# HKUST-SING/herald

Measured on AMD Instinct MI355X. Metric: embedding rows/s (lookup+grad), higher is better.
Workload: dtype f32

## Files before the change

herald_amd/_lib.py:

```python
import ctypes
import os
import re

_PKG = os.path.dirname(os.path.abspath(__file__))
LIB_PATH = os.path.join(_PKG, "libherald_amd.so")
HEADER_PATH = os.path.join(os.path.dirname(_PKG), "include", "herald_amd.h")

_lib = None


class HeraldAmdError(RuntimeError):
    pass


class DLContext(ctypes.Structure):
    _fields_ = [("device_id", ctypes.c_int), ("device_type", ctypes.c_int)]


class DLArray(ctypes.Structure):
    _fields_ = [("data", ctypes.c_void_p), ("ctx", DLContext), ("ndim", ctypes.c_int),
                ("shape", ctypes.POINTER(ctypes.c_int64)), ("stride", ctypes.POINTER(ctypes.c_int64))]


class DLStream(ctypes.Structure):
    _fields_ = [("device_id", ctypes.c_int), ("handle", ctypes.c_void_p)]


class CacheRemote(ctypes.Structure):
    _fields_ = [("req_keys", ctypes.c_void_p), ("req_versions", ctypes.c_void_p), ("inbox_pull", ctypes.c_void_p),
                ("inbox_idx", ctypes.c_void_p), ("inbox_versions", ctypes.c_void_p), ("inbox_rows", ctypes.c_void_p),
                ("out_keys", ctypes.c_void_p), ("out_updates", ctypes.c_void_p), ("out_rows", ctypes.c_void_p),
                ("out_capacity", ctypes.c_int64), ("max_batch", ctypes.c_int64)]


class PlanView(ctypes.Structure):
    _fields_ = [("n", ctypes.c_int64), ("n_unique", ctypes.c_void_p), ("keys", ctypes.c_void_p),
                ("sorted", ctypes.c_void_p), ("perm", ctypes.c_void_p), ("inverse", ctypes.c_void_p),
                ("uniq", ctypes.c_void_p), ("counts", ctypes.c_void_p), ("seg", ctypes.c_void_p),
                ("upos", ctypes.c_void_p)]


def declared_symbols(header=None):
    text = open(header or HEADER_PATH).read()
    text = re.sub(r"/\*.*?\*/", "", text, flags=re.S)
    text = re.sub(r"\(\s*\*\s*\w+\s*\)\s*\([^;{}]*\)\s*;", ";", text)
    names = re.findall(r"\b([A-Za-z_][A-Za-z0-9_]*)\s*\([^;{}]*\)\s*;", text)
    return sorted(set(n for n in names if n not in ("defined", "int", "void", "float")))


PS_LIB_PATH = os.path.join(_PKG, "libherald_ps.so")
PS_HEADER_PATH = os.path.join(os.path.dirname(_PKG), "include", "herald_ps.h")


def load(build_if_missing=True):
    global _lib
    if _lib is not None:
        return _lib
    try:
        import torch
    except ImportError:
        pass
    if not os.path.exists(LIB_PATH):
        if not build_if_missing:
            raise HeraldAmdError("libherald_amd.so is not built (%s)" % LIB_PATH)
        from . import _build
        _build.build_lib()
    try:
        L = ctypes.CDLL(LIB_PATH, mode=ctypes.RTLD_GLOBAL)
    except OSError as e:
        raise HeraldAmdError("cannot load %s: %s" % (LIB_PATH, e))
    _declare(L)
    _lib = L
    return L


class ShardSlot(ctypes.Structure):
    _fields_ = [("world", ctypes.c_int32), ("rank", ctypes.c_int32), ("rcap", ctypes.c_int64), ("n", ctypes.c_int64),
                ("plan_ws", ctypes.c_void_p), ("keys_fixed", ctypes.c_void_p), ("meta_dev", ctypes.c_void_p),
                ("posmap", ctypes.c_void_p), ("rowmap", ctypes.c_void_p), ("counts_host", ctypes.c_void_p),
                ("owner_plan_ws", ctypes.c_void_p)]


def check(rc, what=""):
    if rc != 0:
        msg = load().ha_last_error().decode("utf-8", "replace")
        raise HeraldAmdError("%s failed: %s" % (what or "herald_amd call", msg))


def _declare(L):
    c = ctypes
    vp, i64, f32, sz = c.c_void_p, c.c_int64, c.c_float, c.c_size_t
    L.ha_version.restype = c.c_char_p
    L.ha_last_error.restype = c.c_char_p
    L.ha_device_count.restype = c.c_int
    L.ha_plan_bytes.restype = sz
    L.ha_plan_bytes.argtypes = [i64]
    L.ha_plan_view_of.argtypes = [vp, i64, c.POINTER(PlanView)]
    L.ha_plan_radix_stamps.argtypes = [vp, i64, vp, vp]
    L.ha_pend_bytes.restype = sz
    L.ha_pend_bytes.argtypes = []
    L.ha_plan_handoff_timeout.restype = vp
    L.ha_plan_handoff_timeout.argtypes = [vp]
    L.ha_step_tab_bytes.restype = sz
    L.ha_step_tab_bytes.argtypes = []
    L.ha_step_max_ids.restype = i64
    L.ha_step_max_ids.argtypes = []
    L.ha_qstep_max_ids.restype = i64
    L.ha_qstep_max_ids.argtypes = []
    L.ha_qstep_init.restype = c.c_int
    L.ha_qstep_init.argtypes = []
    L.ha_event_create.restype = vp
    L.ha_event_create.argtypes = []
    L.ha_host_unmap.restype = c.c_int
    L.ha_host_unmap.argtypes = [vp]
    L.ha_qbig_max_ids.restype = i64
    L.ha_qbig_max_ids.argtypes = []
    L.ha_xchg_create.restype = vp
    L.ha_xchg_create.argtypes = [vp, c.c_int, c.c_int]
    L.ha_qbig_plan_bytes.restype = sz
    L.ha_qbig_plan_bytes.argtypes = [i64]
    L.ha_qbig_buckets.restype = c.c_int
    L.ha_qbig_buckets.argtypes = [i64]
    L.ha_qstep_queue_bytes.restype = sz
    L.ha_qstep_queue_bytes.argtypes = [i64, i64]
    L.ha_qstep_queue_header.restype = vp
    L.ha_qstep_queue_header.argtypes = [vp]
    sigs = {
        "ha_gather_f32ids": [vp, i64, i64, vp, i64, vp, vp],
        "ha_gather_u64ids": [vp, i64, i64, vp, i64, vp, vp],
        "ha_gather_u32keys": [vp, i64, i64, vp, i64, vp, vp],
        "ha_scatter_rows_f32ids": [vp, vp, i64, i64, vp, i64, vp],
        "ha_scale_f32": [vp, i64, f32, vp],
        "ha_plan_build_f32ids": [vp, i64, vp, vp],
        "ha_plan_build_u64ids": [vp, i64, vp, vp],
        "ha_plan_build_u32keys": [vp, i64, vp, c.c_int, vp],
        "ha_plan_sort_f32ids": [vp, i64, vp, vp],
        "ha_plan_sort_u32keys": [vp, i64, vp, c.c_int, vp],
        "ha_plan_sort_u64ids": [vp, i64, vp, vp],
        "ha_plan_finish": [vp, i64, vp],
        "ha_plan_build_f32ids_lim": [vp, i64, vp, c.c_uint64, vp],
        "ha_plan_sort_f32ids_lim": [vp, i64, vp, c.c_uint64, vp],
        "ha_plan_build_u64ids_lim": [vp, i64, vp, c.c_uint64, vp],
        "ha_plan_sort_u64ids_lim": [vp, i64, vp, c.c_uint64, vp],
        "ha_plan_export_f32": [vp, i64, vp, vp, vp],
        "ha_dedup_reduce": [vp, i64, vp, i64, vp, vp],
        "ha_apply_mapped": [vp, i64, i64, vp, i64, vp, f32, vp, vp, vp, vp],
        "ha_apply_mapped2": [vp, i64, vp, i64, vp, i64, vp, f32, vp, vp, vp, vp],
        "ha_shard_bucket": [vp, i64, vp, c.c_int, vp, vp, vp],
        "ha_shard_route_f32ids": [vp, i64, vp, vp, c.c_int, vp, vp, vp],
        "ha_shard_route_u64ids": [vp, i64, vp, vp, c.c_int, vp, vp, vp],
        "ha_shard_route_pack_f32ids": [vp, i64, vp, vp, c.c_int, i64, vp, vp, vp],
        "ha_shard_route_pack_u64ids": [vp, i64, vp, vp, c.c_int, i64, vp, vp, vp],
        "ha_shard_route_unpack": [vp, c.c_int, i64, vp, vp, vp],
        "ha_shard_frames_route_f32ids": [vp, i64, vp, vp, c.c_int, i64, i64, vp, vp, vp, vp],
        "ha_shard_frames_route_u64ids": [vp, i64, vp, vp, c.c_int, i64, i64, vp, vp, vp, vp],
        "ha_shard_frames_pack": [vp, i64, vp, c.c_int, i64, i64, vp, vp, vp, vp],
        "ha_shard_frames_unpack": [vp, c.c_int, i64, i64, vp, vp, vp],
        "ha_set_tolerance_mode": [c.c_int],
        "ha_get_tolerance_mode": [],
        "ha_shard_frames_serve_push": [vp, i64, i64, vp, c.c_int, i64, vp, vp, vp],
        "ha_shard_frames_pack_batch": [vp, vp, c.c_int, vp, c.c_int, i64, i64, vp, vp, vp, vp],
        "ha_shard_frames_unpack_batch": [vp, c.c_int, c.c_int, i64, i64, vp, vp, vp],
        "ha_shard_frames_pack_batch_sized": [vp, vp, c.c_int, vp, c.c_int, c.c_int, i64, i64, vp, vp, vp, vp, vp, vp],
        "ha_shard_frames_unpack_batch_sized": [vp, c.c_int, c.c_int, i64, i64, vp, vp, vp, vp],
        "ha_shard_sized_serve_pull": [vp, i64, i64, vp, c.c_int, c.c_int, i64, vp, vp, vp],
        "ha_gather2_u32map": [vp, i64, vp, i64, i64, vp, i64, vp, vp],
        "ha_shard_sized_serve_push": [vp, i64, i64, vp, c.c_int, c.c_int, i64, vp, i64, vp, vp, vp],
        "ha_push_apply_scaled_finished": [vp, i64, i64, vp, i64, vp, f32, vp],
        "ha_qbig_plan_batch_f32ids": [vp, vp, vp, i64, i64, vp],
        "ha_qbig_plan_batch_u64ids": [vp, vp, vp, i64, i64, vp],
        "ha_qbig_queue_batch": [i64, i64, vp, vp, vp, vp, vp, i64, i64, vp, vp, vp],
        "ha_qbig_apply": [vp, i64, i64, vp, i64, vp, f32, vp, i64, vp, vp, i64, i64, c.c_uint32, vp, vp, vp],
        "ha_event_destroy": [vp],
        "ha_event_record": [vp, vp],
        "ha_stream_wait_event": [vp, vp],
        "ha_qqueue_batch_epochs": [i64, i64, vp, vp, vp, vp, vp, i64, i64, vp, vp, vp],
        "ha_shard_step_pull": [vp, i64, i64, vp, vp, vp, vp, i64, vp, vp],
        "ha_shard_step_push": [vp, i64, i64, vp, vp, vp, i64, vp, vp, f32, vp],
        "ha_shard_step": [vp, i64, i64, vp, vp, vp, vp, i64, vp, i64, vp, vp, vp, f32, vp],
        "ha_shard_steps": [vp, i64, i64, i64, vp, vp, vp, vp, i64, vp, i64, vp, vp, vp, f32, vp],
        "ha_qapply_steps_sync": [vp, i64, i64, f32, i64, i64, vp, vp, vp, vp, vp, vp, vp, vp, vp, vp, vp, vp],
        "ha_qapply_steps_counts": [vp, i64, i64, f32, i64, i64, vp, vp, vp, vp, vp, vp, vp, vp, vp, vp, vp, vp, vp],
        "ha_qapply_sync": [vp, i64, i64, vp, i64, vp, f32, vp, i64, vp, vp, i64, i64, c.c_uint32, vp, vp, vp],
        "ha_xchg_available": [],
        "ha_xchg_unique_id": [vp],
        "ha_xchg_destroy": [vp],
        "ha_xchg_bytes": [vp, vp, vp, vp, vp, vp],
        "ha_xchg_rows": [vp, vp, vp, vp, vp, i64, vp],
        "ha_qbig_plan_view": [vp, i64, vp, vp, vp, vp, vp, vp, vp],
        "ha_plan_build_batch_f32ids_lim": [vp, vp, vp, c.c_int, c.c_uint64, vp],
        "ha_plan_sort_batch_f32ids_lim": [vp, vp, vp, c.c_int, c.c_uint64, vp],
        "ha_plan_sort_batch_u64ids_lim": [vp, vp, vp, c.c_int, c.c_uint64, vp],
        "ha_plan_build_batch_u64ids_lim": [vp, vp, vp, c.c_int, c.c_uint64, vp],
        "ha_shard_frames_serve_pull": [vp, i64, i64, vp, c.c_int, i64, i64, vp, vp, vp, vp],
        "ha_shard_serve_push": [vp, i64, i64, vp, i64, vp, vp, vp],
        "ha_dedup_reduce_scaled": [vp, i64, vp, i64, f32, vp, vp],
        "ha_debug_apply_timeline": [vp, i64, i64, vp, i64, vp, f32, vp, vp],
        "ha_sgd_apply": [vp, i64, i64, vp, i64, vp, f32, vp],
        "ha_sgd_apply_finished": [vp, i64, i64, vp, i64, vp, f32, vp],
        "ha_push_apply": [vp, i64, i64, vp, i64, vp, vp],
        "ha_sgd_sparse_update_f32ids": [vp, i64, i64, vp, i64, vp, f32, vp],
        "ha_gather_sum_f32ids": [vp, i64, i64, vp, i64, i64, vp, i64, vp, vp],
        "ha_gather_sum_u64ids": [vp, i64, i64, vp, i64, i64, vp, i64, vp, vp],
        "ha_bag_of": [vp, i64, i64, vp, vp],
        "ha_sgd_apply_bags": [vp, i64, i64, vp, i64, vp, i64, vp, f32, vp],
        "ha_sgd_sparse_update_bags_f32ids": [vp, i64, i64, vp, i64, vp, i64, vp, i64, f32, vp],
        "ha_sgd_sparse_update_bags_u64ids": [vp, i64, i64, vp, i64, vp, i64, vp, i64, f32, vp],
        "ha_debug_bag_slice": [c.c_int],
        "ha_lookup_sort_f32ids": [vp, i64, i64, vp, i64, vp, vp, vp],
        "ha_lookup_sort_u64ids": [vp, i64, i64, vp, i64, vp, vp, vp],
        "ha_sgd_apply_finish": [vp, i64, i64, vp, i64, vp, f32, vp],
        "ha_push_apply_finish": [vp, i64, i64, vp, i64, vp, vp],
        "ha_sgd_apply_finish_prefetch_f32ids": [vp, i64, i64, vp, i64, vp, f32, vp, i64, vp],
        "ha_sparse_opt_fused_f32ids": [c.c_int, vp, i64, i64, vp, i64, vp, vp, vp, vp, vp, vp],
        "ha_pend_reset": [vp, vp],
        "ha_lookup_sort_pend_f32ids": [vp, i64, i64, vp, i64, vp, vp, vp, vp],
        "ha_lookup_sort_pend_u64ids": [vp, i64, i64, vp, i64, vp, vp, vp, vp],
        "ha_sgd_push_pull_f32ids": [vp, i64, i64, vp, i64, vp, f32, vp, vp, i64, vp, vp, vp, vp],
        "ha_sgd_push_pull_u64ids": [vp, i64, i64, vp, i64, vp, f32, vp, vp, i64, vp, vp, vp, vp],
        "ha_step_tab_reset": [vp, vp],
        "ha_step_f32ids": [vp, i64, i64, vp, i64, vp, f32, vp, vp, i64, vp, vp, vp, i64, vp, vp, i64, vp, vp, vp],
        "ha_step_u64ids": [vp, i64, i64, vp, i64, vp, f32, vp, vp, i64, vp, vp, vp, i64, vp, vp, i64, vp, vp, vp],
        "ha_qstep_f32ids": [vp, i64, i64, vp, i64, vp, f32, vp, i64, vp, vp, vp, i64, vp, i64, vp, i64, vp, vp],
        "ha_qstep_u64ids": [vp, i64, i64, vp, i64, vp, f32, vp, i64, vp, vp, vp, i64, vp, i64, vp, i64, vp, vp],
        "ha_qprep_f32ids": [i64, i64, vp, i64, vp, vp, i64, vp, i64, vp, i64, vp],
        "ha_qprep_u64ids": [i64, i64, vp, i64, vp, vp, i64, vp, i64, vp, i64, vp],
        "ha_qplan_batch_f32ids": [vp, vp, vp, i64, vp],
        "ha_qplan_batch_u64ids": [vp, vp, vp, i64, vp],
        "ha_qqueue_batch": [i64, i64, vp, vp, vp, vp, vp, i64, i64, vp],
        "ha_stream_gate": [vp, vp],
        "ha_debug_occupy": [i64, i64, i64, i64, vp],
        "ha_qapply": [vp, i64, i64, vp, i64, vp, f32, vp, i64, vp, vp, i64, vp],
        "ha_qapply_sized": [vp, i64, i64, vp, i64, vp, f32, vp, i64, vp, vp, i64, i64, vp],
        "ha_qapply_steps": [vp, i64, i64, f32, i64, i64, vp, vp, vp, vp, vp, vp, vp, vp, vp],
        "ha_qqueue_batch_counts": [i64, i64, vp, vp, vp, vp, vp, i64, i64, vp, vp],
        "ha_debug_qprep_f32ids": [i64, i64, vp, i64, vp, vp, i64, vp, i64, vp, i64, vp, vp],
        "ha_debug_qapply": [vp, i64, i64, vp, i64, vp, f32, vp, i64, vp, vp, i64, vp, vp],
        "ha_debug_step_fwd_timeline": [vp, i64, i64, vp, i64, vp, f32, vp, vp, i64, vp, vp, vp, i64, vp, vp, i64, vp,
                                       vp, vp, vp],
    }
    for name, args in sigs.items():
        fn = getattr(L, name)
        fn.argtypes = args
        fn.restype = c.c_int
    L.ha_cache_create.restype = vp
    L.ha_cache_create.argtypes = [c.c_int, i64, i64, i64, i64]
    L.ha_cache_destroy.restype = None
    L.ha_cache_destroy.argtypes = [vp]
    for name in ("ha_cache_data", "ha_cache_grad"):
        getattr(L, name).restype = vp
        getattr(L, name).argtypes = [vp]
    for name in ("ha_cache_limit", "ha_cache_width", "ha_cache_fused_updates"):
        getattr(L, name).restype = i64
        getattr(L, name).argtypes = [vp]
    cache_sigs = {
        "ha_cache_set_bounds": [vp, i64, i64],
        "ha_cache_set_bypass": [vp, c.c_int],
        "ha_cache_bind_store": [vp, vp, vp, i64, i64],
        "ha_cache_lookup": [vp, vp, c.c_int, i64, vp, vp],
        "ha_cache_sort_ahead": [vp, vp, c.c_int, i64, vp],
        "ha_cache_lookup_presorted": [vp, vp, c.c_int, i64, vp, vp],
        "ha_cache_sort_ahead_batch": [vp, vp, c.c_int, vp, c.c_int, vp],
        "ha_cache_plan_block": [vp, vp, c.c_int, vp, c.c_int, vp, vp],
        "ha_cache_plan_block_push_keys": [vp, vp, c.c_int, vp, vp, c.c_int, vp, c.c_int, vp, vp],
        "ha_cache_lookup_planned": [vp, i64, vp, vp],
        "ha_cache_update_planned": [vp, i64, vp, vp],
        "ha_cache_plan_pending": [vp],
        "ha_cache_run_planned_pairs": [vp, c.c_int, vp, vp, vp, vp],
        "ha_cache_plan_block_push_pull": [vp, vp, c.c_int, vp, c.c_int, vp, vp],
        "ha_cache_push_pull_planned": [vp, i64, vp, i64, vp, vp],
        "ha_cache_run_planned_push_pulls": [vp, c.c_int, vp, vp, vp, vp, vp],
        "ha_cache_update": [vp, vp, c.c_int, i64, vp, vp],
        "ha_cache_update_same_keys": [vp, i64, vp, vp],
        "ha_cache_update_with_push_keys": [vp, vp, c.c_int, i64, vp, c.c_int, i64, vp, vp],
        "ha_cache_push_pull": [vp, vp, c.c_int, i64, vp, vp, c.c_int, i64, vp, vp],
        "ha_cache_perf": [vp, vp, vp],
        "ha_cache_state": [vp, vp, vp],
        "ha_cache_phase_times": [vp, vp, vp],
        "ha_cache_set_timing": [vp, c.c_int],
        "ha_cache_stage_times": [vp, vp],
        "ha_cache_snapshot": [vp, i64, vp, vp, vp, vp, vp, vp, vp],
        "ha_cache_set_line": [vp, i64, i64, vp, vp],
        "ha_cache_set_remote": [vp],
        "ha_cache_remote_buffers": [vp, vp],
        "ha_cache_lookup_begin": [vp, vp, c.c_int, i64, vp, vp],
        "ha_cache_lookup_finish": [vp, i64, vp, vp],
        "ha_cache_outbox_count": [vp, vp, vp],
        "ha_cache_outbox_pad": [vp, i64],
        "ha_store_count_valid": [vp, i64, i64, vp, vp],
        "ha_cache_push_pull_begin": [vp, vp, c.c_int, i64, vp, c.c_int, i64, vp, vp, vp],
        "ha_cache_push_pull_finish": [vp, vp, vp],
        "ha_store_serve_sync": [vp, vp, i64, i64, vp, vp, i64, i64, vp, vp, vp, vp, vp, vp, vp],
        "ha_store_add_versions": [vp, i64, vp, vp, i64, vp],
        "ha_store_push_distinct": [vp, vp, i64, i64, vp, vp, vp, i64, vp],
    }
    for name, args in cache_sigs.items():
        fn = getattr(L, name)
        fn.argtypes = args
        fn.restype = c.c_int
    L.ha_laia_create.restype = vp
    L.ha_laia_create.argtypes = [vp, i64, i64, i64, i64, i64, i64]
    L.ha_laia_destroy.restype = None
    L.ha_laia_destroy.argtypes = [vp]
    L.ha_laia_next.restype = c.c_int
    L.ha_laia_next.argtypes = [vp, i64, i64, vp, vp, i64, vp]
    L.ha_laia_hint_next.restype = c.c_int
    L.ha_laia_hint_next.argtypes = [vp, i64]
    L.ha_laia_next_for_rank.restype = c.c_int
    L.ha_laia_next_for_rank.argtypes = [vp, i64, i64, i64, vp, vp, i64, vp]
    L.ha_laia_snapshot_keys.restype = i64
    L.ha_laia_snapshot_keys.argtypes = [vp, i64, vp, i64]
    L.ha_laia_next_topk.restype = c.c_int
    L.ha_laia_next_topk.argtypes = [vp, i64, i64, vp, i64, i64, vp, vp, i64, vp]
    L.ha_laia_counters.restype = c.c_int
    L.ha_laia_counters.argtypes = [vp, vp]
    L.ha_laia_timing.restype = c.c_int
    L.ha_laia_timing.argtypes = [vp, vp]
    L.ha_laia_timing_device.restype = c.c_int
    L.ha_laia_timing_device.argtypes = [vp, vp]
    L.ha_laia_on_device.restype = c.c_int
    L.ha_laia_on_device.argtypes = [vp]
    L.ha_shm_ring_open.restype = vp
    L.ha_shm_ring_open.argtypes = [c.c_char_p, c.c_int, i64]
    L.ha_shm_ring_close.restype = None
    L.ha_shm_ring_close.argtypes = [vp]
    L.ha_shm_ring_send.restype = c.c_int
    L.ha_shm_ring_send.argtypes = [vp, vp, i64]
    L.ha_shm_ring_recv.restype = i64
    L.ha_shm_ring_recv.argtypes = [vp, vp, i64, vp]
    L.ha_shm_ring_pending_words.restype = i64
    L.ha_shm_ring_pending_words.argtypes = [vp]
    A, S = c.POINTER(DLArray), c.POINTER(DLStream)
    dl = {
        "DLGpuEmbeddingLookUp": [A, A, A, S],
        "DLGpuEmbeddingLookUp_Gradient": [A, A, A, S],
        "IndexedSlicesOneSideAdd": [A, A, A, S],
        "DeduplicateIndexedSlices": [A, A, A, S],
        "IndexedSlices2Dense": [A, A, A, S],
        "SGDOptimizerSparseUpdate": [A, A, A, f32, S],
        "AdaGradOptimizerSparseUpdate": [A, A, A, A, f32, f32, S],
        "AdamOptimizerSparseUpdate": [A, A, A, A, A, f32, f32, f32, f32, f32, f32, S],
        "AdamWOptimizerSparseUpdate": [A, A, A, A, A, f32, f32, f32, f32, f32, f32, f32, S],
        "AddL2RegularizationSparse": [A, A, A, f32, S],
        "MomentumOptimizerSparseUpdate": [A, A, A, A, f32, f32, c.c_bool, S],
        "LambOptimizerSparseUpdate": [A, A, A, A, A, f32, f32, f32, f32, f32, f32, f32, S],
        "cpu_EmbeddingLookup": [A, A, A],
        "cpu_SGDOptimizerSparseUpdate": [A, A, A, f32],
    }
    for name, args in dl.items():
        fn = getattr(L, name)
        fn.argtypes = args
        fn.restype = c.c_int
```

herald_amd/csrc/qstep.hip:

```cpp
#include <hip/hip_ext.h>

#include "plan_dev.h"
#include "gather_dev.h"

namespace ha {

constexpr int kQMax = 7168;
#ifndef QV_GOLD
#define QV_GOLD 1
#endif
#ifndef QV_WG
#define QV_WG (QV_GOLD ? 1024 : 256)
#endif
#ifndef QV_COOPSLOTS
#define QV_COOPSLOTS (QV_GOLD ? 64 : 256)
#endif
constexpr int kQWg = QV_WG;
constexpr int kQWpw = kQWg / 64;
constexpr int kQCoopSlots = QV_COOPSLOTS;
constexpr int kQWorkerMax = 448 * 16 / kQWpw;
constexpr int kQSmallC = 3, kQSmallM = 16, kQMediumC = 15, kQLongC = 64;
enum QKind { kQS = 0, kQM = 1, kQL = 2, kQZ = 3, kQG = 4, kQNone = 15 };

struct QHeader {
// ... 1988 lines not shown
    HA_REQUIRE(rows >= 0 && rows <= 0xFFFFFFFEll && width >= 4 && width % 4 == 0 && width <= (1 << 20),
               "ha_qbig_queue_batch: rows of a multiple of 4 floats");
    HA_REQUIRE(count >= 0 && (count == 0 || (ws_a && n_a && ws_g && n_g && queues)), "ha_qbig_queue_batch: null pointer");
    HA_REQUIRE(n_cap >= 1 && n_cap <= kQBigMax, "ha_qbig_queue_batch: bad capacity");
    static DeviceOnce lds_allowed;
    if (lds_allowed.run([]() -> int {
            HA_ALLOW_LDS(qbqueue_kernel<true>, 160 * 1024);
            HA_ALLOW_LDS(qbqueue_kernel<false>, 160 * 1024);
            return 0;
        }))
        return -1;
    const int P = qbig_buckets(n_cap);
    for (int64_t k0 = 0; k0 < count; k0 += kQJoinBatch) {
        QBigJoinBatch b;
        QBigZero z;
        memset(&b, 0, sizeof(b));
        memset(&z, 0, sizeof(z));
        b.rows = static_cast<uint64_t>(rows);
        b.width = static_cast<int>(width);
        b.P = P;
        for (int64_t k = k0; k < count && b.count < kQJoinBatch; ++k) {
            HA_REQUIRE(n_a[k] >= 0 && n_g[k] >= 0 && n_a[k] <= n_cap && n_g[k] <= n_cap,
                       "ha_qbig_queue_batch: a batch is larger than the queues were sized for");
            if (n_a[k] == 0 && n_g[k] == 0)
                continue;
            HA_REQUIRE(queues[k] && (n_a[k] == 0 || ws_a[k]) && (n_g[k] == 0 || ws_g[k]),
                       "ha_qbig_queue_batch: null pointer (step %lld)", (long long)k);
            const int i = b.count++;
            if (n_a[k] > 0)
                qbig_layout(ws_a[k], n_cap, &b.a[i]);
            if (n_g[k] > 0)
                qbig_layout(ws_g[k], n_cap, &b.g[i]);
            b.a[i].n = static_cast<int>(n_a[k]);
            b.g[i].n = static_cast<int>(n_g[k]);
            const QLayout q = queue_layout(queues[k], n_cap, width);
            b.qh[i] = q.hdr;
            z.qh[z.count++] = q.hdr;
            b.mirror[i] = counts_host ? counts_host[k] : nullptr;
            b.epoch[i] = epochs ? epochs[k] : 0u;
            b.coop[i] = q.coop;
            b.wave[i] = q.wave;
            b.copy[i] = q.copy;
            b.cap_coop = q.cap_coop;
            b.cap_wave = q.cap_wave;
            b.cap_copy = q.cap_copy;
        }
        if (b.count == 0)
            continue;
        const size_t need = qjoin_lds_bytes(kQMax, kQMax), res = qjoin_lds_resident_bytes(kQMax);
        const size_t lds1 = need > res ? need : res;
        b.lds_bytes = static_cast<uint32_t>(lds1);
        hipLaunchKernelGGL(qbzero_kernel, dim3(z.count), dim3(64), 0, stream, z);
        HA_LAUNCH_CHECK();
        hipLaunchKernelGGL(qbqueue_kernel<true>, dim3(2 * (P / 4), b.count), dim3(1024), 4 * kQSubJoinLds, stream, b);
        hipLaunchKernelGGL(qbqueue_kernel<false>, dim3(2 * (P / 4), b.count), dim3(1024), lds1, stream, b);
        HA_LAUNCH_CHECK();
    }
    return 0;
}

}

using namespace ha;

extern "C" int64_t ha_qstep_max_ids(void) { return kQMax; }

extern "C" int ha_qstep_init(void) {
    const float *ids = nullptr;
    const uint64_t *ids64 = nullptr;
    if (qplan_batch<float>(&ids, nullptr, nullptr, 0, nullptr) || qplan_batch<uint64_t>(&ids64, nullptr, nullptr, 0, nullptr) ||
        qqueue_batch(0, 4, nullptr, nullptr, nullptr, nullptr, nullptr, 1, 0, nullptr))
        return -1;
    return lds_atomics_lane_ordered();
}

extern "C" size_t ha_qstep_queue_bytes(int64_t n_cap, int64_t width) {
    if (n_cap < 1 || width < 4)
        return 0;
    return queue_layout(nullptr, n_cap, width).bytes;
}

extern "C" int ha_qplan_batch_f32ids(const float *const *ids, const int64_t *n, void *const *plans, int64_t count,
                                     ha_stream_t stream) {
    return qplan_batch<float>(ids, n, plans, count, as_stream(stream));
}
extern "C" int ha_qplan_batch_u64ids(const uint64_t *const *ids, const int64_t *n, void *const *plans, int64_t count,
                                     ha_stream_t stream) {
    return qplan_batch<uint64_t>(ids, n, plans, count, as_stream(stream));
}
extern "C" int ha_qqueue_batch(int64_t rows, int64_t width, void *const *plans_a, const int64_t *n_a,
                               void *const *plans_g, const int64_t *n_g, void *const *queues, int64_t queue_n_cap,
                               int64_t count, ha_stream_t stream) {
    return qqueue_batch(rows, width, plans_a, n_a, plans_g, n_g, queues, queue_n_cap, count, as_stream(stream));
}
extern "C" int ha_qapply(float *table, int64_t rows, int64_t width, void *plan_cur, int64_t n_cur, const float *grads,
                         float lr, void *plan_next, int64_t n_next, float *next_out, const void *queue_cur,
                         int64_t queue_n_cap, ha_stream_t stream) {
    return qapply(table, rows, width, plan_cur, n_cur, grads, lr, plan_next, n_next, next_out, queue_cur, queue_n_cap,
                  as_stream(stream));
}
extern "C" int ha_qapply_sized(float *table, int64_t rows, int64_t width, void *plan_cur, int64_t n_cur, const float *grads,
                               float lr, void *plan_next, int64_t n_next, float *next_out, const void *queue_cur,
                               int64_t queue_n_cap, int64_t wave_items, ha_stream_t stream) {
    return qapply(table, rows, width, plan_cur, n_cur, grads, lr, plan_next, n_next, next_out, queue_cur, queue_n_cap,
                  as_stream(stream), nullptr, wave_items);
}
extern "C" int ha_qapply_steps(float *table, int64_t rows, int64_t width, float lr, int64_t queue_n_cap, int64_t count,
                               void *const *plan_cur, const int64_t *n_cur, const float *const *grads,
                               void *const *plan_next, const int64_t *n_next, float *const *next_out,
                               const void *const *queue_cur, const int64_t *wave_items, ha_stream_t stream) {
    HA_REQUIRE(count >= 0 && (count == 0 || (plan_cur && n_cur && grads && plan_next && n_next && next_out && queue_cur)),
               "ha_qapply_steps: null pointer");
    for (int64_t k = 0; k < count; ++k)
        if (qapply(table, rows, width, plan_cur[k], n_cur[k], grads[k], lr, plan_next[k], n_next[k], next_out[k],
                   queue_cur[k], queue_n_cap, as_stream(stream), nullptr, wave_items ? wave_items[k] : -1))
            return -1;
    return 0;
}

extern "C" void *ha_event_create(void) {
    hipEvent_t e = nullptr;
    if (hipEventCreateWithFlags(&e, hipEventDisableTiming) != hipSuccess)
        return nullptr;
    return e;
}
extern "C" int ha_event_destroy(void *event) {
    if (event)
        HA_CHECK_HIP(hipEventDestroy(static_cast<hipEvent_t>(event)));
    return 0;
}
extern "C" int ha_event_record(void *event, ha_stream_t stream) {
    HA_REQUIRE(event != nullptr, "ha_event_record: null event");
    HA_CHECK_HIP(hipEventRecord(static_cast<hipEvent_t>(event), as_stream(stream)));
    return 0;
}
extern "C" int ha_stream_wait_event(ha_stream_t stream, void *event) {
    HA_REQUIRE(event != nullptr, "ha_stream_wait_event: null event");
    HA_CHECK_HIP(hipStreamWaitEvent(as_stream(stream), static_cast<hipEvent_t>(event), 0));
    return 0;
}
extern "C" int ha_qqueue_batch_epochs(int64_t rows, int64_t width, void *const *plans_a, const int64_t *n_a,
                                      void *const *plans_g, const int64_t *n_g, void *const *queues, int64_t queue_n_cap,
                                      int64_t count, uint32_t *const *counts_host, const uint32_t *epochs,
                                      ha_stream_t stream) {
    return qqueue_batch(rows, width, plans_a, n_a, plans_g, n_g, queues, queue_n_cap, count, as_stream(stream), nullptr,
                        counts_host, epochs);
}
extern "C" int ha_qapply_steps_sync(float *table, int64_t rows, int64_t width, float lr, int64_t queue_n_cap, int64_t count,
                                    void *const *plan_cur, const int64_t *n_cur, const float *const *grads,
                                    void *const *plan_next, const int64_t *n_next, float *const *next_out,
                                    const void *const *queue_cur, const int64_t *wave_items, const uint32_t *epochs,
                                    uint32_t *err, void *done_event, ha_stream_t stream) {
    HA_REQUIRE(count >= 0 && (count == 0 || (plan_cur && n_cur && grads && plan_next && n_next && next_out && queue_cur)),
               "ha_qapply_steps_sync: null pointer");
    for (int64_t k = 0; k < count; ++k)
        if (qapply(table, rows, width, plan_cur[k], n_cur[k], grads[k], lr, plan_next[k], n_next[k], next_out[k],
                   queue_cur[k], queue_n_cap, as_stream(stream), nullptr, wave_items ? wave_items[k] : -1,
                   epochs ? epochs[k] : 0u, err, k + 1 == count ? static_cast<hipEvent_t>(done_event) : nullptr))
            return -1;
    if (count == 0 && done_event)
        HA_CHECK_HIP(hipEventRecord(static_cast<hipEvent_t>(done_event), as_stream(stream)));
    return 0;
}
extern "C" int ha_qapply_steps_counts(float *table, int64_t rows, int64_t width, float lr, int64_t queue_n_cap, int64_t count,
                                      void *const *plan_cur, const int64_t *n_cur, const float *const *grads,
                                      void *const *plan_next, const int64_t *n_next, float *const *next_out,
                                      const void *const *queue_cur, const int64_t *wave_items,
                                      const uint32_t *const *counts_host, const uint32_t *epochs, uint32_t *err,
                                      void *done_event, ha_stream_t stream) {
    (void)counts_host;
    return ha_qapply_steps_sync(table, rows, width, lr, queue_n_cap, count, plan_cur, n_cur, grads, plan_next, n_next, next_out,
                                queue_cur, wave_items, epochs, err, done_event, stream);
}
extern "C" int ha_qapply_sync(float *table, int64_t rows, int64_t width, void *plan_cur, int64_t n_cur, const float *grads,
                              float lr, void *plan_next, int64_t n_next, float *next_out, const void *queue_cur,
                              int64_t queue_n_cap, int64_t wave_items, uint32_t epoch, uint32_t *err, void *done_event,
                              ha_stream_t stream) {
    return qapply(table, rows, width, plan_cur, n_cur, grads, lr, plan_next, n_next, next_out, queue_cur, queue_n_cap,
                  as_stream(stream), nullptr, wave_items, epoch, err, static_cast<hipEvent_t>(done_event));
}

extern "C" int ha_qqueue_batch_counts(int64_t rows, int64_t width, void *const *plans_a, const int64_t *n_a,
                                      void *const *plans_g, const int64_t *n_g, void *const *queues, int64_t queue_n_cap,
                                      int64_t count, uint32_t *const *counts_host, ha_stream_t stream) {
    return qqueue_batch(rows, width, plans_a, n_a, plans_g, n_g, queues, queue_n_cap, count, as_stream(stream), nullptr,
                        counts_host);
}

template <typename IdT>
static int qprep_one(int64_t rows, int64_t width, const IdT *ahead_ids, int64_t n_ahead, void *plan_ahead, void *plan_a,
                     int64_t n_a, void *plan_g, int64_t n_g, void *queue_build, int64_t queue_n_cap, hipStream_t s) {
    if (n_ahead > 0 && qplan_batch<IdT>(&ahead_ids, &n_ahead, &plan_ahead, 1, s))
        return -1;
    if (n_a > 0 || n_g > 0)
        return qqueue_batch(rows, width, &plan_a, &n_a, &plan_g, &n_g, &queue_build, queue_n_cap, 1, s);
    return 0;
}
extern "C" int ha_qprep_f32ids(int64_t rows, int64_t width, const float *ahead_ids, int64_t n_ahead, void *plan_ahead,
                               void *plan_a, int64_t n_a, void *plan_g, int64_t n_g, void *queue_build,
                               int64_t queue_n_cap, ha_stream_t stream) {
    return qprep_one<float>(rows, width, ahead_ids, n_ahead, plan_ahead, plan_a, n_a, plan_g, n_g, queue_build,
                            queue_n_cap, as_stream(stream));
}
extern "C" int ha_qprep_u64ids(int64_t rows, int64_t width, const uint64_t *ahead_ids, int64_t n_ahead, void *plan_ahead,
                               void *plan_a, int64_t n_a, void *plan_g, int64_t n_g, void *queue_build,
                               int64_t queue_n_cap, ha_stream_t stream) {
    return qprep_one<uint64_t>(rows, width, ahead_ids, n_ahead, plan_ahead, plan_a, n_a, plan_g, n_g, queue_build,
                               queue_n_cap, as_stream(stream));
}
extern "C" int ha_qstep_f32ids(float *table, int64_t rows, int64_t width, void *plan_cur, int64_t n_cur,
                               const float *grads, float lr, void *plan_next, int64_t n_next, float *next_out,
                               const void *queue_cur, void *plan_b1, int64_t n_b1, void *queue_build,
                               int64_t queue_n_cap, const float *ahead_ids, int64_t n_ahead, void *plan_ahead,
                               ha_stream_t stream) {
    if (qprep_one<float>(rows, width, ahead_ids, n_ahead, plan_ahead, plan_next, n_next, plan_b1, n_b1, queue_build,
                         queue_n_cap, as_stream(stream)))
        return -1;
    return qapply(table, rows, width, plan_cur, n_cur, grads, lr, plan_next, n_next, next_out, queue_cur, queue_n_cap,
                  as_stream(stream));
}
extern "C" int ha_qstep_u64ids(float *table, int64_t rows, int64_t width, void *plan_cur, int64_t n_cur,
                               const float *grads, float lr, void *plan_next, int64_t n_next, float *next_out,
                               const void *queue_cur, void *plan_b1, int64_t n_b1, void *queue_build,
                               int64_t queue_n_cap, const uint64_t *ahead_ids, int64_t n_ahead, void *plan_ahead,
                               ha_stream_t stream) {
    if (qprep_one<uint64_t>(rows, width, ahead_ids, n_ahead, plan_ahead, plan_next, n_next, plan_b1, n_b1, queue_build,
                            queue_n_cap, as_stream(stream)))
        return -1;
    return qapply(table, rows, width, plan_cur, n_cur, grads, lr, plan_next, n_next, next_out, queue_cur, queue_n_cap,
                  as_stream(stream));
}

extern "C" int64_t ha_qbig_max_ids(void) { return kQBigMax; }
extern "C" size_t ha_qbig_plan_bytes(int64_t n_cap) {
    if (n_cap < 1 || n_cap > kQBigMax)
        return 0;
    return qbig_layout(nullptr, n_cap, nullptr);
}
extern "C" int ha_qbig_buckets(int64_t n_cap) { return n_cap >= 1 && n_cap <= kQBigMax ? qbig_buckets(n_cap) : 0; }
extern "C" int ha_qbig_plan_batch_f32ids(const float *const *ids, const int64_t *n, void *const *ws, int64_t n_cap,
                                         int64_t count, ha_stream_t stream) {
    return qbig_plan_batch<float>(ids, n, ws, n_cap, count, as_stream(stream));
}
extern "C" int ha_qbig_plan_batch_u64ids(const uint64_t *const *ids, const int64_t *n, void *const *ws, int64_t n_cap,
                                         int64_t count, ha_stream_t stream) {
    return qbig_plan_batch<uint64_t>(ids, n, ws, n_cap, count, as_stream(stream));
}
extern "C" int ha_qbig_queue_batch(int64_t rows, int64_t width, void *const *ws_a, const int64_t *n_a, void *const *ws_g,
                                   const int64_t *n_g, void *const *queues, int64_t n_cap, int64_t count,
                                   uint32_t *const *counts_host, const uint32_t *epochs, ha_stream_t stream) {
    return qbig_queue_batch(rows, width, ws_a, n_a, ws_g, n_g, queues, n_cap, count, counts_host, epochs, as_stream(stream));
}
extern "C" int ha_qbig_apply(float *table, int64_t rows, int64_t width, void *ws_cur, int64_t n_cur, const float *grads,
                             float lr, void *ws_next, int64_t n_next, float *next_out, const void *queue_cur, int64_t n_cap,
                             int64_t coop_items, uint32_t epoch, uint32_t *err, void *done_event, ha_stream_t stream) {
    HA_REQUIRE(n_cap >= 1 && n_cap <= kQBigMax && (n_cur == 0 || ws_cur) && (n_next == 0 || ws_next), "ha_qbig_apply: bad arguments");
    QBigRef a, g;
    memset(&a, 0, sizeof(a));
    memset(&g, 0, sizeof(g));
    if (n_cur > 0)
        qbig_layout(ws_cur, n_cap, &a);
    if (n_next > 0)
        qbig_layout(ws_next, n_cap, &g);
    return qapply_lists(table, rows, width, a.gperm, n_cur, grads, lr, g.gperm, n_next, next_out, queue_cur, n_cap, kQBigMax,
                        as_stream(stream), nullptr, -1, epoch, err, static_cast<hipEvent_t>(done_event), coop_items);
}
extern "C" int ha_qbig_plan_view(void *ws, int64_t n_cap, void **boff, void **bhdr, void **uniq, void **counts, void **seg,
                                 void **gperm, void **meta) {
    HA_REQUIRE(ws && n_cap >= 1 && n_cap <= kQBigMax, "ha_qbig_plan_view: bad arguments");
    QBigRef r;
    qbig_layout(ws, n_cap, &r);
    if (boff) *boff = r.boff;
    if (bhdr) *bhdr = r.bhdr;
    if (uniq) *uniq = r.uniq;
    if (counts) *counts = r.counts;
    if (seg) *seg = r.seg;
    if (gperm) *gperm = r.gperm;
    if (meta) *meta = r.meta;
    return 0;
}

extern "C" int ha_debug_qapply(float *table, int64_t rows, int64_t width, void *plan_cur, int64_t n_cur,
                               const float *grads, float lr, void *plan_next, int64_t n_next, float *next_out,
                               const void *queue_cur, int64_t queue_n_cap, unsigned long long *dbg, ha_stream_t stream) {
    HA_REQUIRE(dbg != nullptr, "qapply timeline: null debug buffer");
    return qapply(table, rows, width, plan_cur, n_cur, grads, lr, plan_next, n_next, next_out, queue_cur, queue_n_cap,
                  as_stream(stream), dbg);
}
extern "C" int ha_debug_qprep_f32ids(int64_t rows, int64_t width, const float *ahead_ids, int64_t n_ahead,
                                     void *plan_ahead, void *plan_a, int64_t n_a, void *plan_g, int64_t n_g,
                                     void *queue_build, int64_t queue_n_cap, unsigned long long *ph, ha_stream_t stream) {
    HA_REQUIRE(ph != nullptr, "qprep phases: null debug buffer");
    if (n_ahead > 0 && qplan_batch<float>(&ahead_ids, &n_ahead, &plan_ahead, 1, as_stream(stream), ph))
        return -1;
    if (n_a > 0 || n_g > 0)
        return qqueue_batch(rows, width, &plan_a, &n_a, &plan_g, &n_g, &queue_build, queue_n_cap, 1, as_stream(stream),
                            ph + 16);
    return 0;
}

extern "C" const uint32_t *ha_qstep_queue_header(const void *queue) {
    return reinterpret_cast<const uint32_t *>(queue);
}
```

herald_amd/ops.py:

```python
import ctypes
import os

import numpy as np

import torch

from . import _lib
from ._lib import DLArray, DLContext, DLStream, PlanView, check


def _stream_ptr(stream=None):
    if stream is None:
        return ctypes.c_void_p(torch._C._cuda_getCurrentRawStream(torch.cuda.current_device()))
    if isinstance(stream, int):
        return ctypes.c_void_p(stream)
    return ctypes.c_void_p(stream.cuda_stream)


def _ptr(t):
    return ctypes.c_void_p(t.data_ptr())


def _raw_stream(stream=None):
    p = _stream_ptr(stream).value
# ... 404 lines not shown
    L = _lib.load()
    _require(table, torch.float32, "table")
    n = ids.numel()
    width = table.shape[1]
    if n > plan.capacity:
        raise ValueError("plan capacity %d < %d ids" % (plan.capacity, n))
    if out is None:
        out = torch.empty(tuple(ids.shape) + (width,), dtype=torch.float32, device=table.device)
    fn = getattr(L, "ha_lookup_sort_pend_" + _ids_kind(ids))
    check(fn(_ptr(table), table.shape[0], width, _ptr(ids), n, _ptr(out), _ptr(plan.ws), _ptr(pend.buf),
             _stream_ptr(stream)), "ha_lookup_sort_pend")
    plan.n = n
    plan._view = None
    plan.produced_on(stream)
    return out


def sgd_push_pull(table, plan_cur, grads, lr, pend_cur, next_ids=None, plan_next=None, pend_next=None,
                  next_out=None, stream=None):
    L = _lib.load()
    _require(table, torch.float32, "table")
    _require(grads, torch.float32, "grads")
    width = table.shape[1]
    if next_ids is None:
        check(L.ha_sgd_push_pull_f32ids(_ptr(table), table.shape[0], width, _ptr(plan_cur.ws), plan_cur.n,
                                        _ptr(grads), ctypes.c_float(lr), _ptr(pend_cur.buf), None, 0, None,
                                        None, None, _stream_ptr(stream)), "ha_sgd_push_pull")
        plan_cur.produced_on(stream)
        return None
    n = next_ids.numel()
    if n > plan_next.capacity:
        raise ValueError("plan capacity %d < %d ids" % (plan_next.capacity, n))
    if next_out is None:
        next_out = torch.empty(tuple(next_ids.shape) + (width,), dtype=torch.float32, device=table.device)
    fn = getattr(L, "ha_sgd_push_pull_" + _ids_kind(next_ids))
    check(fn(_ptr(table), table.shape[0], width, _ptr(plan_cur.ws), plan_cur.n, _ptr(grads),
             ctypes.c_float(lr), _ptr(pend_cur.buf), _ptr(next_ids), n, _ptr(next_out), _ptr(plan_next.ws),
             _ptr(pend_next.buf), _stream_ptr(stream)), "ha_sgd_push_pull")
    plan_next.n = n
    plan_next._view = None
    plan_cur.produced_on(stream)
    plan_next.produced_on(stream)
    return next_out


def check_handoff(plans):
    for p in plans:
        p._sync_producer()
        p._raise_if_handoff_timed_out()


class SortAhead:

    def __init__(self, table, capacity, lr, device=None):
        _require(table, torch.float32, "table")
        self.table, self.lr = table, float(lr)
        self.device = table.device if device is None else torch.device(device)
        self.plans = [IndexPlan(capacity, self.device), IndexPlan(capacity, self.device)]
        self.side = torch.cuda.Stream(device=self.device)
        self.k = 0
        self.plan = None

    def _sort(self, plan, ids):
        cur = torch.cuda.current_stream(self.device)
        self.side.wait_stream(cur)
        plan.sort(ids.reshape(-1), stream=self.side, key_limit=self.table.shape[0])

    def begin(self, ids0):
        self.k = 0
        self._sort(self.plans[0], ids0)
        torch.cuda.current_stream(self.device).wait_stream(self.side)

    def lookup(self, ids, next_ids=None, out=None):
        if next_ids is not None:
            self._sort(self.plans[(self.k + 1) % 2], next_ids)
        return embedding_lookup(self.table, ids, out=out)

    def apply(self, grads):
        cur = torch.cuda.current_stream(self.device)
        plan = self.plans[self.k % 2]
        sgd_apply_finish(self.table, plan, grads, self.lr)
        cur.wait_stream(self.side)
        self.plan = plan
        self.k += 1
        return plan


def step_max_ids():
    return int(_lib.load().ha_step_max_ids())


class StepPipeline:

    NPLAN, NTAB = 4, 4

    def __init__(self, table, capacity, lr, device=None):
        L = _lib.load()
        _require(table, torch.float32, "table")
        self.table, self.lr = table, float(lr)
        self.device = table.device if device is None else torch.device(device)
        if capacity > step_max_ids():
            raise ValueError("ha_step_* takes at most %d ids per batch (got capacity %d): use sgd_push_pull / "
                             "lookup_sort + sgd_apply_finish" % (step_max_ids(), capacity))
        self.capacity = capacity
        self.plans = [IndexPlan(capacity, self.device) for _ in range(self.NPLAN)]
        self.tab_bytes = int(L.ha_step_tab_bytes())
        self.tabs = torch.empty(self.NTAB * self.tab_bytes, dtype=torch.uint8, device=self.device)
        self.c = None
        self.n = {}
        self.shape = {}
        self.reset()

    def _tab(self, c):
        return self.tabs.data_ptr() + (c % self.NTAB) * self.tab_bytes

    def plan_of(self, c):
        return self.plans[c % self.NPLAN]

    def reset(self, stream=None):
        L = _lib.load()
        for t in range(self.NTAB):
            check(L.ha_step_tab_reset(self._tab(t), _stream_ptr(stream)), "ha_step_tab_reset")
        if stream is None:
            torch.cuda.current_stream(self.device).synchronize()
        self.c, self.n, self.shape = None, {}, {}
        return self

    def launch(self, c, n_cur, grads, n_next, out, n_fin, ahead_ids, stream=None):
        L = _lib.load()
        t = self.table
        width = t.shape[1]
        n_ahead = 0 if ahead_ids is None else ahead_ids.numel()
        if max(n_cur, n_next, n_fin, n_ahead) > self.capacity:
            raise ValueError("plan capacity %d < %d ids" % (self.capacity, max(n_cur, n_next, n_fin, n_ahead)))
        if n_cur:
            _require(grads, torch.float32, "grads")
            if grads.numel() != n_cur * width:
                raise ValueError("grads must hold %d x %d values" % (n_cur, width))
        if n_next:
            _require(out, torch.float32, "out")
            if out.numel() != n_next * width:
                raise ValueError("out must hold %d x %d values" % (n_next, width))
        kind = _ids_kind(ahead_ids) if n_ahead else "f32ids"
        fn = getattr(L, "ha_step_" + kind)
        check(fn(_ptr(t), t.shape[0], width,
                 _ptr(self.plan_of(c).ws) if n_cur else None, n_cur, _ptr(grads) if n_cur else None,
                 ctypes.c_float(self.lr), self._tab(c) if n_cur else None,
                 _ptr(self.plan_of(c + 1).ws) if n_next else None, n_next, _ptr(out) if n_next else None,
                 self._tab(c + 1) if n_next else None,
                 _ptr(self.plan_of(c + 2).ws) if n_fin else None, n_fin, self._tab(c + 2) if n_fin else None,
                 _ptr(ahead_ids) if n_ahead else None, n_ahead,
                 _ptr(self.plan_of(c + 3).ws) if n_ahead else None,
                 self._tab(c + 3), _stream_ptr(stream)), "ha_step")
        if n_fin:
            self.plan_of(c + 2).produced_on(stream)
        if n_ahead:
            pl = self.plan_of(c + 3)
            pl.n = n_ahead
            pl._view = None
            pl.produced_on(stream)

    def _call(self, c, grads, ahead_ids, out, stream):
        n_cur, n_next, n_fin = self.n.get(c, 0), self.n.get(c + 1, 0), self.n.get(c + 2, 0)
        n_ahead = 0 if ahead_ids is None else ahead_ids.numel()
        if n_next and out is None:
            out = torch.empty(tuple(self.shape[c + 1]) + (self.table.shape[1],), dtype=torch.float32,
                              device=self.table.device)
        self.launch(c, n_cur, grads, n_next, out, n_fin, ahead_ids, stream)
        if n_cur:
            del self.n[c]
        if n_ahead:
            self.n[c + 3] = n_ahead
            self.shape[c + 3] = tuple(ahead_ids.shape)
        self.c = c + 1
        return out if n_next else None

    def start(self, ids0, ids1=None, ids2=None, out=None, stream=None):
        self._call(-3, None, ids0, None, stream)
        self._call(-2, None, ids1, None, stream)
        return self._call(-1, None, ids2, out, stream)

    def step(self, grads, ahead_ids=None, out=None, stream=None):
        if self.c is None or self.c not in self.n:
            raise RuntimeError("StepPipeline.step without a batch in flight (call start first)")
        return self._call(self.c, grads, ahead_ids, out, stream)


def qbig_max_ids():
    return int(_lib.load().ha_qbig_max_ids())


class WidePlan:

    def __init__(self, capacity, device):
        L = _lib.load()
        self.capacity, self.device = int(capacity), device
        self.ws = torch.zeros(int(L.ha_qbig_plan_bytes(self.capacity)), dtype=torch.uint8, device=device)
        torch.cuda.current_stream(device).synchronize()
        self.buckets = int(L.ha_qbig_buckets(self.capacity))
        self.n = 0
        self._produced_on, self._view = 0, None

    def groups(self):
        L = _lib.load()
        ptr = [ctypes.c_void_p() for _ in range(7)]
        check(L.ha_qbig_plan_view(_ptr(self.ws), self.capacity, *[ctypes.byref(p) for p in ptr]), "ha_qbig_plan_view")
        torch.cuda.synchronize(self.device)
        base = self.ws.data_ptr()

        def arr(p, count, dtype):
            off = p.value - base
            return self.ws[off:off + count * dtype.itemsize].view(dtype).cpu().numpy()
        P, n = self.buckets, self.n
        boff = arr(ptr[0], P + 1, torch.int32).astype(np.int64)
        hdr = arr(ptr[1], P * 32, torch.int64).reshape(P, 32)
        uniq = arr(ptr[2], max(n, 1), torch.int32).astype(np.int64) & 0xFFFFFFFF
        counts = arr(ptr[3], max(n, 1), torch.int32).astype(np.int64)
        gperm = arr(ptr[5], max(n, 1), torch.int32).astype(np.int64)
        meta = arr(ptr[6], 1, torch.int32)
        keys, cnts, lists = [], [], []
        for p in range(P):
            U = int(hdr[p, 0])
            o = int(boff[p])
            keys.append(uniq[o:o + U])
            cnts.append(counts[o:o + U])
            lists.append(gperm[o:int(boff[p + 1])])
        return {"overflow": int(meta[0]), "bucket_sizes": np.diff(boff), "uniq": np.concatenate(keys) if keys else uniq[:0],
                "counts": np.concatenate(cnts) if cnts else counts[:0], "perm": np.concatenate(lists) if lists else gperm[:0]}


def qstep_max_ids():
    return int(_lib.load().ha_qstep_max_ids())


class SortAheadPipeline:

    NBLOCKS = 3

    def __init__(self, table, max_ids, lr, block=8, key_limit=None, device=None, finish_ahead=None):
        _require(table, torch.float32, "table")
        self.table, self.lr, self.block = table, float(lr), int(block)
        self.device = table.device if device is None else torch.device(device)
        self.key_limit = int(table.shape[0]) if key_limit is None else int(key_limit)
        self.finish_ahead = bool(finish_ahead)
        self.plans = [[IndexPlan(max_ids, self.device) for _ in range(self.block)] for _ in range(self.NBLOCKS)]
        self.side = torch.cuda.Stream(device=self.device)
        self._sorted = [torch.cuda.Event() for _ in range(self.NBLOCKS)]
        self._freed = [None] * self.NBLOCKS
        self._first = [0] * self.NBLOCKS
        self._count = [0] * self.NBLOCKS
        self._next_block = 0
        self._waited = -1

    def prepare_block(self, ids_list):
        if not 0 < len(ids_list) <= self.block:
            raise ValueError("a block holds 1..%d batches" % self.block)
        b = self._next_block
        slot = b % self.NBLOCKS
        self.side.wait_stream(torch.cuda.current_stream(self.device))
        with torch.cuda.stream(self.side):
            if self._freed[slot] is not None:
                self.side.wait_event(self._freed[slot])
            for i, ids in enumerate(ids_list):
                if self.finish_ahead:
                    self.plans[slot][i].build(ids, stream=self.side, key_limit=self.key_limit)
                else:
                    self.plans[slot][i].sort(ids, stream=self.side, key_limit=self.key_limit)
            self._sorted[slot].record(self.side)
        self._first[slot] = (self._first[(b - 1) % self.NBLOCKS] + self._count[(b - 1) % self.NBLOCKS]) if b else 0
        self._count[slot] = len(ids_list)
        self._next_block = b + 1
        return b

    def _plan(self, k, stream):
        for b in range(max(self._next_block - self.NBLOCKS, 0), self._next_block):
            slot = b % self.NBLOCKS
            if self._first[slot] <= k < self._first[slot] + self._count[slot]:
                if b > self._waited:
                    (stream or torch.cuda.current_stream(self.device)).wait_event(self._sorted[slot])
                    self._waited = b
                return slot, k - self._first[slot]
        raise ValueError("step %d is not in a prepared block" % k)

    def lookup(self, k, ids, out=None, stream=None):
        self._plan(k, stream)
        return embedding_lookup(self.table, ids, out=out, stream=stream)

    def apply(self, k, grads, stream=None):
        slot, i = self._plan(k, stream)
        if self.finish_ahead:
            sgd_apply(self.table, self.plans[slot][i], grads, self.lr, stream=stream, finished=True)
            self.plans[slot][i].produced_on(self.side)
        else:
            sgd_apply_finish(self.table, self.plans[slot][i], grads, self.lr, stream=stream)
        if i == self._count[slot] - 1:
            ev = torch.cuda.Event()
            ev.record(stream or torch.cuda.current_stream(self.device))
            self._freed[slot] = ev
        return self.plans[slot][i]


class QueueStepPipeline:

    def __init__(self, table, capacity, lr, device=None, block=8, overlap=True, sync="events", min_flags_block=8):
        L = _lib.load()
        _require(table, torch.float32, "table")
        self.table, self.lr = table, float(lr)
        self.device = table.device if device is None else torch.device(device)
        self.wide = capacity > qstep_max_ids()
        if capacity > qbig_max_ids():
            raise ValueError("ha_qstep_* takes at most %d ids per batch (got capacity %d): use SortAheadPipeline / "
                             "lookup_sort + sgd_apply_finish" % (qbig_max_ids(), capacity))
        if table.shape[1] % 4 != 0:
            raise ValueError("ha_qstep_* needs rows of a multiple of 4 floats")
        with torch.cuda.device(self.device):
            if L.ha_qstep_init() < 0:
                check(-1, "ha_qstep_init")
        self.capacity = max(int(capacity), 1)
        self.overlap = bool(overlap)
        if sync not in ("events", "flags"):
            raise ValueError("sync must be 'events' or 'flags'")
        self.sync = sync if self.overlap else "events"
        if self.sync == "flags" and int(block) < int(min_flags_block):
            self.sync = "events"
        self._done_ev, self._cev_pool = {}, []
        self._cev_busy = []
        self.block = int(block) if self.overlap else 1
        if not 1 <= self.block <= 64:
            raise ValueError("block must be 1..64")
        self.LOOKAHEAD = 3 * self.block
        self.NPLAN, self.NQUEUE = 4 * self.block, 2 * self.block
        self.ROTATION = 4 * self.block
        self.plans = [(WidePlan if self.wide else IndexPlan)(self.capacity, self.device) for _ in range(self.NPLAN)]
        self.queue_bytes = int(L.ha_qstep_queue_bytes(self.capacity, table.shape[1]))
        self.queues = torch.zeros(self.NQUEUE * self.queue_bytes, dtype=torch.uint8, device=self.device)
        torch.cuda.current_stream(self.device).synchronize()
        side_prio = 0
        if os.environ.get("HA_QSIDE_PRIO") in ("low", "high"):
            try:
                lo_hi = torch.cuda.Stream.priority_range()
                side_prio = max(lo_hi) if os.environ["HA_QSIDE_PRIO"] == "low" else min(lo_hi)
            except Exception:
                side_prio = 0
        self.side = torch.cuda.Stream(device=self.device, priority=side_prio) if self.overlap else None
        self.COUNTS = 8192
        self.counts = torch.zeros((self.COUNTS, 4), dtype=torch.int32).pin_memory()
        self._counts_np = self.counts.numpy()
        self._counts_c = (ctypes.c_int32 * (self.COUNTS * 4)).from_address(self.counts.data_ptr())
        self._counts_base = self.counts.data_ptr()
        self._L = L
        self._plan_ptr = [p.ws.data_ptr() for p in self.plans]
        self._queue_ptr = [self.queues.data_ptr() + q * self.queue_bytes for q in range(self.NQUEUE)]
        self._ev_pool = []
        self._last_items = 0
        self.fallbacks, self._fb_plan, self._wide_ids = 0, None, {}
        self._enq_last = None
        self.reset()

    def close(self):
        for ev in list(self._done_ev.values()) + self._cev_pool + [e for e, _ in self._cev_busy]:
            self._L.ha_event_destroy(ev)
        self._done_ev, self._cev_pool, self._cev_busy = {}, [], []

    def __del__(self):
        try:
            self.close()
        except Exception:
            pass

    def reset(self, stream=None):
        if self._done_ev:
            if self.side is not None:
                marker = self._event() if hasattr(self, "_ev_pool") else torch.cuda.Event()
                marker.record(self.side)
                self._cev_busy.extend((e, marker) for e in self._done_ev.values())
            else:
                self._cev_pool.extend(self._done_ev.values())
        self._done_ev = {}
        self.c, self.n, self.shape, self.ids = None, {}, {}, {}
        self._enq_last, self._covered = None, -(1 << 60)
        self._ev_side = {}
        self._held = {}
        return self

    def plan_of(self, b):
        return self.plans[b % self.NPLAN]

    def _queue(self, c):
        return self.queues.data_ptr() + (c % self.NQUEUE) * self.queue_bytes

    def queue_header(self, c):
        off = (c % self.NQUEUE) * self.queue_bytes
        torch.cuda.synchronize(self.device)
        h = self.queues[off:off + 40].view(torch.int32).cpu().tolist()
        d = dict(zip(("wave_items", "workgroup_items", "long", "medium", "small", "copy_items"), h))
        d["overflow"] = int(h[8] != 0 or h[9] != 0)
        return d

    def overflowed(self):
        return bool((self._counts_np[:, 3] & ~4).any())

    def _raise_if_failed(self, steps):
        cc, ring = self._counts_c, self.COUNTS
        for j in steps:
            f = cc[4 * (j % ring) + 3]
            if f & ~4:
                raise RuntimeError("QueueStepPipeline: step %d failed on the device (flags %d: 1 = queue overflow, 2 = an "
                                   "occurrence list out of position order, 8 = an apply launch gave up waiting -- its queue was "
                                   "never completed, or an item it depends on never finished; the table is partly updated)"
                                   % (j, f))

    def prepare_block(self, b, ids_of, stream=None, ph=None):
        L = self._L
        rows, width = self.table.shape
        main = stream if stream is not None else torch.cuda.current_stream(self.device)
        B = self.block
        s = self.side if self.overlap else main
        sp = _stream_ptr(s)
        vp, i64 = ctypes.c_void_p, ctypes.c_int64
        flags = self.sync == "flags"
        self._raise_if_failed(range(max((b - 2) * B, 0), max((b - 1) * B, 0)))
        if self.overlap and flags:
            cev = self._done_ev.pop(b - 1, None)
            if cev is not None:
                check(L.ha_stream_wait_event(sp, cev), "ha_stream_wait_event")
                marker = self._event()
                marker.record(s)
                self._cev_busy.append((cev, marker))
                self._covered = b * B - 1
            elif self._enq_last is not None and self._enq_last > self._covered:
                ev = self._event()
                ev.record(main)
                s.wait_event(ev)
                self._ev_pool.append(ev)
                self._covered = self._enq_last
        elif self.overlap:
            ev = self._event()
            ev.record(main)
            s.wait_event(ev)
        sel = {"f32ids": [], "u64ids": []}
        held = []
        for j in range((b + 2) * B, (b + 3) * B):
            t = ids_of(j)
            if t is None:
                continue
            m = t.numel()
            if m == 0:
                continue
            if m > self.capacity:
                raise ValueError("plan capacity %d < %d ids" % (self.capacity, m))
            if not t.is_cuda or not t.is_contiguous():
                raise ValueError("ids must be contiguous device tensors")
            sel[_ids_kind(t)].append((j, t, m))
            held.append(t)
            self.n[j] = m
            if self.wide:
                self._wide_ids[j] = t
                self._wide_ids.pop(j - 5 * B, None)
        for kind, lst in sel.items():
            if not lst:
                continue
            cnt = len(lst)
            ids_arr = (vp * cnt)(*[t.data_ptr() for _, t, _ in lst])
            n_arr = (i64 * cnt)(*[m for _, _, m in lst])
            pl_arr = (vp * cnt)(*[self._plan_ptr[j % self.NPLAN] for j, _, _ in lst])
            if ph is not None and kind == "f32ids":
                j0, t0, m0 = lst[0]
                check(L.ha_debug_qprep_f32ids(rows, width, _ptr(t0), m0, _ptr(self.plan_of(j0).ws), None, 0,
                                              None, 0, None, self.capacity, _ptr(ph), sp), "ha_debug_qprep")
            if self.wide:
                check(getattr(L, "ha_qbig_plan_batch_" + kind)(ids_arr, n_arr, pl_arr, self.capacity, cnt, sp),
                      "ha_qbig_plan_batch")
            else:
                check(getattr(L, "ha_qplan_batch_" + kind)(ids_arr, n_arr, pl_arr, cnt, sp), "ha_qplan_batch")
            for j, _, m in lst:
                pl = self.plans[j % self.NPLAN]
                pl.n = m
                pl._view = None
                pl._produced_on = sp.value if sp.value is not None else 0
        self._held[b] = held
        self._held.pop(b - 2, None)
        nget = self.n.get
        steps = [j for j in range((b + 1) * B, (b + 2) * B) if nget(j, 0) or nget(j + 1, 0)]
        if steps:
            cnt = len(steps)
            pp, NP, NQ = self._plan_ptr, self.NPLAN, self.NQUEUE
            pa = (vp * cnt)(*[pp[j % NP] if nget(j, 0) else None for j in steps])
            na = (i64 * cnt)(*[nget(j, 0) for j in steps])
            pg = (vp * cnt)(*[pp[(j + 1) % NP] if nget(j + 1, 0) else None for j in steps])
            ng = (i64 * cnt)(*[nget(j + 1, 0) for j in steps])
            qs = (vp * cnt)(*[self._queue_ptr[j % NQ] for j in steps])
            if ph is not None:
                check(L.ha_debug_qprep_f32ids(rows, width, None, 0, None, pa[0], na[0], pg[0], ng[0], qs[0], self.capacity,
                                              _ptr(ph), sp), "ha_debug_qprep")
            base, ring, cc = self._counts_base, self.COUNTS, self._counts_c
            for j in steps:
                at = 4 * (j % ring)
                cc[at] = 0
                cc[at + 2] = 0
                cc[at + 3] &= ~4
            cs = (vp * cnt)(*[base + 16 * (j % ring) for j in steps])
            eps = (ctypes.c_uint32 * cnt)(*[self._epoch(j) for j in steps])
            if self.wide:
                check(L.ha_qbig_queue_batch(rows, width, pa, na, pg, ng, qs, self.capacity, cnt, cs, eps, sp),
                      "ha_qbig_queue_batch")
            else:
                check(L.ha_qqueue_batch_epochs(rows, width, pa, na, pg, ng, qs, self.capacity, cnt, cs, eps, sp),
                      "ha_qqueue_batch")
        if self.overlap and not flags:
            ev = self._event()
            ev.record(s)
            self._ev_side[b] = ev
            ready = self._ev_side.pop(b - 1, None)
            if ready is not None:
                main.wait_event(ready)
                self._ev_pool.append(ready)

    def _event(self):
        return self._ev_pool.pop() if self._ev_pool else torch.cuda.Event()

    @staticmethod
    def _epoch(j):
        return (j + (1 << 24)) & 0xFFFFFFFF

    def _block_done_event(self, c):
        if self.sync != "flags" or (c + 1) % self.block != 0:
            return None
        if not self._cev_pool and self._cev_busy and self._cev_busy[0][1].query():
            old_ev, marker = self._cev_busy.pop(0)
            self._ev_pool.append(marker)
            self._cev_pool.append(old_ev)
        ev = self._cev_pool.pop() if self._cev_pool else ctypes.c_void_p(self._L.ha_event_create())
        if not ev:
            raise RuntimeError("ha_event_create failed")
        old = self._done_ev.pop(c // self.block, None)
        if old is not None:
            self._cev_pool.append(old)
        self._done_ev[c // self.block] = ev
        return ev

    def _err_ptr(self, c):
        return ctypes.c_void_p(self._counts_base + 16 * (c % self.COUNTS) + 12)

    def wave_items(self, c):
        at = 4 * (c % self.COUNTS)
        if self._counts_c[at + 3]:
            raise RuntimeError("ha_qqueue_batch: the work queue of step %d is unusable (flags %d: 1 = overflow, 2 = an "
                               "occurrence list out of position order, 4 = a hash bucket of a wide batch holds more than "
                               "%d ids)" % (c, self._counts_c[at + 3], qstep_max_ids()))
        if os.environ.get("HA_QHINT") == "0":
            return -1
        w, cp = self._counts_c[at], self._counts_c[at + 2]
        return w + cp - 2 if w > 0 and cp > 0 else -1

    def apply(self, c, grads, out, stream=None, dbg=None, n_cur=None, n_next=None):
        L = self._L
        t = self.table
        rows, width = t.shape
        n_cur = self.n.get(c, 0) if n_cur is None else int(n_cur)
        n_next = self.n.get(c + 1, 0) if n_next is None else int(n_next)
        if n_cur:
            _require(grads, torch.float32, "grads")
            if grads.numel() != n_cur * width:
                raise ValueError("grads must hold %d x %d values" % (n_cur, width))
        if n_next:
            _require(out, torch.float32, "out")
            if out.numel() != n_next * width:
                raise ValueError("out must hold %d x %d values" % (n_next, width))
        flags = self.sync == "flags" and dbg is None
        capturing = flags and torch.cuda.is_current_stream_capturing()
        if capturing:
            raise RuntimeError("QueueStepPipeline(sync='flags'): steps cannot be captured into a hipGraph (use sync='events')")
        done = self._block_done_event(c) if flags else None
        self._enq_last = c if self._enq_last is None else max(self._enq_last, c)
        if not (n_cur or n_next):
            if done is not None:
                check(L.ha_event_record(done, _stream_ptr(stream)), "ha_event_record")
            return
        args = [_ptr(t), rows, width, _ptr(self.plan_of(c).ws) if n_cur else None, n_cur,
                _ptr(grads) if n_cur else None, ctypes.c_float(self.lr),
                _ptr(self.plan_of(c + 1).ws) if n_next else None, n_next, _ptr(out) if n_next else None,
                self._queue(c), self.capacity]
        if self.wide:
            flag, coop = self._wide_built(c)
            if flag & 4:
                self._wide_fallback(c, grads, out, stream, n_cur, n_next, done)
                return
            if flag:
                self.wave_items(c)
            check(L.ha_qbig_apply(*args, coop, self._epoch(c) if flags else 0, self._err_ptr(c) if flags else None, done,
                                  _stream_ptr(stream)), "ha_qbig_apply")
        elif flags:
            check(L.ha_qapply_sync(*args, self.wave_items(c), self._epoch(c), self._err_ptr(c), done, _stream_ptr(stream)),
                  "ha_qapply_sync")
        elif dbg is None:
            check(L.ha_qapply_sized(*args, self.wave_items(c), _stream_ptr(stream)), "ha_qapply")
        else:
            check(L.ha_debug_qapply(*args, _ptr(dbg), _stream_ptr(stream)), "ha_debug_qapply")

    def _wide_built(self, c, timeout=20.0):
        import time
        at = 4 * (c % self.COUNTS)
        cc = self._counts_c
        if cc[at] == 0:
            t0 = time.perf_counter()
            while cc[at] == 0:
                if time.perf_counter() - t0 > timeout:
                    raise RuntimeError("QueueStepPipeline: the queue of step %d was not built within %.0f s (was its block "
                                       "prepared?)" % (c, timeout))
        return cc[at + 3], max(cc[at + 1] - 1, 0)

    def _wide_fallback(self, c, grads, out, stream, n_cur, n_next, done):
        self.fallbacks += 1
        if n_cur:
            if self._fb_plan is None:
                self._fb_plan = IndexPlan(self.capacity, self.device)
            self._fb_plan.build(self._wide_ids[c], stream=stream)
            sgd_apply(self.table, self._fb_plan, grads.reshape(n_cur, -1), self.lr, stream=stream, finished=True)
        if n_next:
            embedding_lookup(self.table, self._wide_ids[c + 1].reshape(-1), out=out.reshape(n_next, -1), stream=stream)
        if done is not None:
            check(self._L.ha_event_record(done, _stream_ptr(stream)), "ha_event_record")

    def apply_call(self, c, grads, out, stream, n_cur, n_next, sized=True):
        if self.sync == "flags":
            raise RuntimeError("apply_call: use apply / apply_steps_call with sync='flags'")
        L = self._L
        t = self.table
        rows, width = t.shape
        hint = ctypes.c_int64(-1)
        args = (ctypes.c_void_p(t.data_ptr()), ctypes.c_int64(rows), ctypes.c_int64(width),
                ctypes.c_void_p(self.plan_of(c).ws.data_ptr() if n_cur else None), ctypes.c_int64(n_cur),
                ctypes.c_void_p(grads.data_ptr() if n_cur else None), ctypes.c_float(self.lr),
                ctypes.c_void_p(self.plan_of(c + 1).ws.data_ptr() if n_next else None), ctypes.c_int64(n_next),
                ctypes.c_void_p(out.data_ptr() if n_next else None), ctypes.c_void_p(self._queue(c)),
                ctypes.c_int64(self.capacity), hint, _stream_ptr(stream))
        fn = L.ha_qapply_sized

        def call(k):
            self._enq_last = k if self._enq_last is None else max(self._enq_last, k)
            if sized:
                hint.value = self.wave_items(k)
            if fn(*args) != 0:
                check(-1, "ha_qapply")
        return call

    def apply_steps_call(self, c0, grads_list, out_list, stream, n, sized=True):
        L = self._L
        t = self.table
        rows, width = t.shape
        cnt = len(grads_list)
        vp, i64 = ctypes.c_void_p, ctypes.c_int64
        pc = (vp * cnt)(*[self.plan_of(c0 + i).ws.data_ptr() for i in range(cnt)])
        pn = (vp * cnt)(*[self.plan_of(c0 + i + 1).ws.data_ptr() for i in range(cnt)])
        ns = (i64 * cnt)(*[n] * cnt)
        gs = (vp * cnt)(*[g.data_ptr() for g in grads_list])
        os_ = (vp * cnt)(*[o.data_ptr() for o in out_list])
        qs = (vp * cnt)(*[self._queue(c0 + i) for i in range(cnt)])
        hints = (i64 * cnt)(*[-1] * cnt)
        head = (vp(t.data_ptr()), i64(rows), i64(width), ctypes.c_float(self.lr), i64(self.capacity), i64(cnt))
        sp = _stream_ptr(stream)
        fn = L.ha_qapply_steps
        counts, ring = self._counts_c, self.COUNTS
        flags = self.sync == "flags"
        eps = (ctypes.c_uint32 * cnt)()
        fn_sync, epoch, last_err = L.ha_qapply_steps_counts, self._epoch, self._err_ptr
        B = self.block
        cs = (vp * cnt)()
        base = self._counts_base
        use_counts = os.environ.get("HA_QCOUNTS", "0") != "0"

        def call(k0):
            if flags and k0 // B != (k0 + cnt - 1) // B:
                raise RuntimeError("apply_steps_call(sync='flags'): steps %d..%d cross a block boundary (block = %d)"
                                   % (k0, k0 + cnt - 1, B))
            self._enq_last = k0 + cnt - 1 if self._enq_last is None else max(self._enq_last, k0 + cnt - 1)
            if sized:
                for i in range(cnt):
                    at = 4 * ((k0 + i) % ring)
                    w, cp = counts[at], counts[at + 2]
                    if counts[at + 3]:
                        raise RuntimeError("ha_qqueue_batch: the work queue of step %d is unusable (flags %d: 1 = overflow, "
                                           "2 = an occurrence list out of position order)" % (k0 + i, counts[at + 3]))
                    if w > 0 and cp > 0:
                        self._last_items = w + cp - 2
                    hints[i] = w + cp - 2 if w > 0 and cp > 0 else (self._last_items * 17) // 16 if self._last_items > 0 else -1
                    cs[i] = base + 4 * at if use_counts else None
            if flags:
                for i in range(cnt):
                    eps[i] = epoch(k0 + i)
                done = self._block_done_event(k0 + cnt - 1)
                if fn_sync(*head, pc, ns, gs, pn, ns, os_, qs, hints, cs if sized else None, eps, last_err(k0 + cnt - 1), done,
                           sp) != 0:
                    check(-1, "ha_qapply_steps_counts")
            elif fn(*head, pc, ns, gs, pn, ns, os_, qs, hints, sp) != 0:
                check(-1, "ha_qapply_steps")
        return call

    def _call(self, c, grads, ahead_ids, out, stream):
        if c % self.block == 0:
            self.prepare_block(c // self.block, lambda j: self.ids.get(j), stream)
            for j in [j for j in self.ids if j < c + 3 * self.block]:
                del self.ids[j]
        if ahead_ids is not None and ahead_ids.numel():
            self.ids[c + self.LOOKAHEAD] = ahead_ids
            self.shape[c + self.LOOKAHEAD] = tuple(ahead_ids.shape)
        n_next = self.n.get(c + 1, 0)
        if n_next and out is None:
            out = torch.empty(tuple(self.shape[c + 1]) + (self.table.shape[1],), dtype=torch.float32,
                              device=self.table.device)
        self.apply(c, grads, out, stream)
        for d in (self.n, self.shape):
            d.pop(c - 1, None)
        self.c = c + 1
        return out if n_next else None

    def start(self, ids, out=None, stream=None):
        ids = list(ids)
        if len(ids) > self.LOOKAHEAD:
            raise ValueError("start takes the first %d batches" % self.LOOKAHEAD)
        ids = ids + [None] * (self.LOOKAHEAD - len(ids))
        self.reset()
        res = None
        for k, b in enumerate(ids):
            c = k - self.LOOKAHEAD
            res = self._call(c, None, b, out if c == -1 else None, stream)
        return res

    def step(self, grads, ahead_ids=None, out=None, stream=None):
        if self.c is None:
            raise RuntimeError("QueueStepPipeline.step before start")
        return self._call(self.c, grads, ahead_ids, out, stream)


def push_apply_finish(table, plan, grads, stream=None):
    _require(table, torch.float32, "table")
    _require(grads, torch.float32, "grads")
    check(_lib.load().ha_push_apply_finish(_ptr(table), table.shape[0], table.shape[1], _ptr(plan.ws),
                                           plan.n, _ptr(grads), _stream_ptr(stream)),
          "ha_push_apply_finish")
    plan.produced_on(stream)
    return table


def dl_call(name, arrays, scalars=(), stream=None):
    L = _lib.load()
    holders = [DLHolder(a) for a in arrays]
    sh = DLStreamHolder(stream)
    args = [h.handle for h in holders] + list(scalars) + [sh.handle]
    check(getattr(L, name)(*args), name)


class IndexedSlices:

    def __init__(self, indices=None, values=None, dense_shape=None, push_indices=None, bag=None, bag_of=None):
        if bag is not None and bag_of is not None:
            raise ValueError("give at most one of bag and bag_of")
        self.indices = indices
        self.values = values
        self.dense_shape = dense_shape
        self.push_indices = push_indices
        self.bag, self.bag_of = bag, bag_of
        self.deduplicated = False

    @property
    def pooled(self):
        return self.bag is not None or self.bag_of is not None

    def expanded_values(self, stream=None):
        width = self.values.shape[-1]
        vals = self.values.reshape(-1, width).contiguous()
        if not self.pooled:
            return vals
        n = self.indices.numel()
        if self.bag is not None:
            rows = torch.arange(n, dtype=torch.int64, device=vals.device) // int(self.bag)
        else:
            rows = self.bag_of.reshape(-1).to(torch.int64)
        return embedding_lookup(vals, rows, stream=stream)

    def get_dense_shape(self):
        assert self.dense_shape is not None
        return self.dense_shape

    def get_sparse_shape(self):
        return tuple(self.values.shape)

    def update(self, indices, values, dense_shape, push_indices=None, bag=None, bag_of=None):
        self.indices = indices
        self.push_indices = push_indices
        self.bag, self.bag_of = bag, bag_of
        self.values = values
        if self.dense_shape is not None:
            assert tuple(self.dense_shape) == tuple(dense_shape)
        else:
            self.dense_shape = dense_shape
        self.deduplicated = False

    def deduplicate(self, stream=None):
        if self.pooled:
            raise ValueError("pooled IndexedSlices (bag / bag_of) cannot be deduplicated: values holds one row per bag")
        ids = self.indices.reshape(-1)
        n = ids.numel()
        width = self.values.shape[-1]
        plan = IndexPlan(max(n, 1), device=ids.device).build(ids, stream)
        reduced = dedup_reduce(plan, self.values.reshape(n, width), stream=stream)
        uniq_f32, _ = plan.export_f32(stream)
        u = uniq_f32.numel()
        self.indices = uniq_f32
        self.values = reduced[:u]
        if self.push_indices is not None:
            pids = self.push_indices.reshape(-1)
            pplan = IndexPlan(max(pids.numel(), 1), device=pids.device).build(pids, stream)
            self.push_indices, _ = pplan.export_f32(stream)
        self.deduplicated = True
        return self

    def to_dense(self, stream=None):
        if self.pooled:
            raise ValueError("pooled IndexedSlices (bag / bag_of) have no dense form: values holds one row per bag")
        dense = torch.zeros(tuple(self.get_dense_shape()), dtype=torch.float32, device=self.values.device)
        dl_call("IndexedSlices2Dense", [self.values.contiguous(), self.indices.contiguous(), dense],
                stream=stream)
        return dense
```

include/herald_amd.h:

```cpp
#ifndef HERALD_AMD_H_
#define HERALD_AMD_H_

#include <stddef.h>
#include <stdint.h>

#ifdef __cplusplus
extern "C" {
#endif

typedef enum { kCPU = 1, kGPU = 2 } DLDeviceType;
typedef struct {
    int device_id;
    DLDeviceType device_type;
} DLContext;
typedef struct {
    void *data;
    DLContext ctx;
    int ndim;
    int64_t *shape;
    int64_t *stride;
} DLArray;
typedef struct {
    int device_id;
    void *handle;
} DLStream;
typedef DLArray *DLArrayHandle;
typedef DLStream *DLStreamHandle;

typedef void *ha_stream_t;

const char *ha_version(void);
const char *ha_last_error(void);
int ha_scratch_release(void);
int ha_device_count(void);


int DLGpuEmbeddingLookUp(const DLArrayHandle input, const DLArrayHandle ids,
                         DLArrayHandle output, DLStreamHandle stream_handle);

int DLGpuEmbeddingLookUp_Gradient(const DLArrayHandle output_grad,
                                  const DLArrayHandle ids,
                                  DLArrayHandle input_grad,
                                  DLStreamHandle stream_handle);

int IndexedSlicesOneSideAdd(const DLArrayHandle indices,
                            const DLArrayHandle values, DLArrayHandle output,
                            DLStreamHandle stream_handle);

int DeduplicateIndexedSlices(const DLArrayHandle origin,
                             const DLArrayHandle inverse,
                             DLArrayHandle compressed,
                             DLStreamHandle stream_handle);

int IndexedSlices2Dense(const DLArrayHandle values, const DLArrayHandle indices,
                        DLArrayHandle new_values, DLStreamHandle stream_handle);

int SGDOptimizerSparseUpdate(DLArrayHandle param,
                             const DLArrayHandle grad_indices,
                             const DLArrayHandle grad_values, float lr,
                             DLStreamHandle stream_handle);

int AdaGradOptimizerSparseUpdate(DLArrayHandle param,
                                 const DLArrayHandle grad_indices,
                                 const DLArrayHandle grad_values,
                                 DLArrayHandle acc, float lr, float eps,
                                 DLStreamHandle stream_handle);
int AdamOptimizerSparseUpdate(DLArrayHandle param,
                              const DLArrayHandle grad_indices,
                              const DLArrayHandle grad_values,
                              DLArrayHandle expavg, DLArrayHandle expavgsq,
                              float lr, float beta1, float beta2, float beta1t,
                              float beta2t, float eps,
                              DLStreamHandle stream_handle);
int AdamWOptimizerSparseUpdate(DLArrayHandle param,
                               const DLArrayHandle grad_indices,
                               const DLArrayHandle grad_values,
                               DLArrayHandle expavg, DLArrayHandle expavgsq,
                               float lr, float beta1, float beta2,
                               float beta1t, float beta2t, float eps,
                               float weight_decay,
                               DLStreamHandle stream_handle);
int AddL2RegularizationSparse(const DLArrayHandle param,
                              const DLArrayHandle grad_indices,
                              DLArrayHandle grad_values, float l2reg,
                              DLStreamHandle stream_handle);
int MomentumOptimizerSparseUpdate(DLArrayHandle param,
                                  const DLArrayHandle grad_indices,
                                  const DLArrayHandle grad_values,
                                  DLArrayHandle velocity, float lr,
                                  float momentum, bool nesterov,
                                  DLStreamHandle stream_handle);
int LambOptimizerSparseUpdate(DLArrayHandle param,
                              const DLArrayHandle grad_indices,
                              const DLArrayHandle grad_values,
                              DLArrayHandle expavg, DLArrayHandle expavgsq,
                              float lr, float beta1, float beta2, float beta1t,
                              float beta2t, float eps, float weight_decay,
                              DLStreamHandle stream_handle);
int ha_host_unmap(void *host_array);
int cpu_EmbeddingLookup(const DLArrayHandle in_mat, const DLArrayHandle ids,
                        DLArrayHandle out_mat);
int cpu_SGDOptimizerSparseUpdate(DLArrayHandle param,
                                 const DLArrayHandle grad_indices,
                                 const DLArrayHandle grad_values, float lr);


int ha_set_tolerance_mode(int on);
int ha_get_tolerance_mode(void);

int ha_gather_f32ids(const float *table, int64_t rows, int64_t width,
                     const float *ids, int64_t n, float *out,
                     ha_stream_t stream);
int ha_gather_u64ids(const float *table, int64_t rows, int64_t width,
                     const uint64_t *ids, int64_t n, float *out,
                     ha_stream_t stream);
int ha_gather_u32keys(const float *table, int64_t rows, int64_t width,
                      const uint32_t *keys, int64_t n, float *out,
                      ha_stream_t stream);

int ha_scatter_rows_f32ids(const float *values, const float *ids, int64_t n,
                           int64_t width, float *dst, int64_t rows,
                           ha_stream_t stream);

int ha_scale_f32(float *values, int64_t n, float scale, ha_stream_t stream);

typedef struct {
    int64_t n;
    int64_t *n_unique;
    uint32_t *keys;
    uint32_t *sorted;
    int32_t *perm;
    int32_t *inverse;
    uint32_t *uniq;
    int32_t *counts;
    int32_t *seg;
    int32_t *upos;
} ha_plan_view;

size_t ha_plan_bytes(int64_t n);
int ha_plan_view_of(void *ws, int64_t n, ha_plan_view *view);
int ha_plan_radix_stamps(void *ws, int64_t n, uint64_t *out_host, ha_stream_t stream);
int ha_plan_build_f32ids(const float *ids, int64_t n, void *ws,
                         ha_stream_t stream);
int ha_plan_build_u64ids(const uint64_t *ids, int64_t n, void *ws,
                         ha_stream_t stream);
int ha_plan_sort_u32keys(const uint32_t *keys, int64_t n, void *plan_ws, int key_bits, ha_stream_t stream);
int ha_plan_sort_f32ids(const float *ids, int64_t n, void *ws,
                        ha_stream_t stream);
int ha_plan_sort_u64ids(const uint64_t *ids, int64_t n, void *ws,
                        ha_stream_t stream);
int ha_plan_build_batch_f32ids_lim(const float *const *ids, const int64_t *n, void *const *ws, int count,
                                   uint64_t key_limit, ha_stream_t stream);
int ha_plan_build_batch_u64ids_lim(const uint64_t *const *ids, const int64_t *n, void *const *ws, int count,
                                   uint64_t key_limit, ha_stream_t stream);
int ha_plan_sort_batch_f32ids_lim(const float *const *ids, const int64_t *n, void *const *ws, int count,
                                  uint64_t key_limit, ha_stream_t stream);
int ha_plan_sort_batch_u64ids_lim(const uint64_t *const *ids, const int64_t *n, void *const *ws, int count,
                                  uint64_t key_limit, ha_stream_t stream);
int ha_plan_build_f32ids_lim(const float *ids, int64_t n, void *ws, uint64_t key_limit, ha_stream_t stream);
int ha_plan_sort_f32ids_lim(const float *ids, int64_t n, void *ws, uint64_t key_limit, ha_stream_t stream);
int ha_plan_build_u64ids_lim(const uint64_t *ids, int64_t n, void *ws, uint64_t key_limit, ha_stream_t stream);
int ha_plan_sort_u64ids_lim(const uint64_t *ids, int64_t n, void *ws, uint64_t key_limit, ha_stream_t stream);
int ha_plan_finish(void *ws, int64_t n, ha_stream_t stream);
int ha_plan_build_u32keys(const uint32_t *keys, int64_t n, void *ws,
                          int key_bits, ha_stream_t stream);
int ha_plan_export_f32(const void *ws, int64_t n, float *uniq_f32,
                       float *inverse_f32, ha_stream_t stream);

int ha_dedup_reduce(const void *plan_ws, int64_t n, const float *grads,
                    int64_t width, float *reduced, ha_stream_t stream);

int ha_dedup_reduce_scaled(const void *plan_ws, int64_t n, const float *grads,
                           int64_t width, float scale, float *reduced,
                           ha_stream_t stream);

int ha_sgd_apply(float *table, int64_t rows, int64_t width,
                 const void *plan_ws, int64_t n, const float *grads, float lr,
                 ha_stream_t stream);
int ha_sgd_apply_finished(float *table, int64_t rows, int64_t width, void *plan_ws, int64_t n, const float *grads,
                          float lr, ha_stream_t stream);

int ha_push_apply(float *table, int64_t rows, int64_t width,
                  const void *plan_ws, int64_t n, const float *grads,
                  ha_stream_t stream);

int ha_apply_mapped(float *dst, int64_t dst_rows, int64_t width,
                    const void *plan_ws, int64_t n, const float *src, float lr,
                    const int32_t *rowmap, const int32_t *valmap,
                    const uint8_t *dst_init, ha_stream_t stream);
int ha_apply_mapped2(float *dst, int64_t dst_rows, float *dst2, int64_t width,
                     const void *plan_ws, int64_t n, const float *src, float lr,
                     const int32_t *rowmap, const int32_t *rowmap2,
                     const uint8_t *dst_init, ha_stream_t stream);

int ha_sparse_opt_fused_f32ids(int kind, float *param, int64_t rows, int64_t width, const float *ids,
                               int64_t n, const float *grads, float *state1, float *state2,
                               const float *hyper_host, void *plan_ws, ha_stream_t stream);

int ha_lookup_sort_f32ids(const float *table, int64_t rows, int64_t width,
                          const float *ids, int64_t n, float *out,
                          void *plan_ws, ha_stream_t stream);
int ha_lookup_sort_u64ids(const float *table, int64_t rows, int64_t width,
                          const uint64_t *ids, int64_t n, float *out,
                          void *plan_ws, ha_stream_t stream);
int ha_sgd_apply_finish(float *table, int64_t rows, int64_t width,
                        void *plan_ws, int64_t n, const float *grads, float lr,
                        ha_stream_t stream);
int ha_push_apply_finish(float *table, int64_t rows, int64_t width,
                         void *plan_ws, int64_t n, const float *grads,
                         ha_stream_t stream);

size_t ha_pend_bytes(void);
int ha_pend_reset(void *pend, ha_stream_t stream);
int ha_lookup_sort_pend_f32ids(const float *table, int64_t rows, int64_t width,
                               const float *ids, int64_t n, float *out,
                               void *plan_ws, void *pend, ha_stream_t stream);
int ha_lookup_sort_pend_u64ids(const float *table, int64_t rows, int64_t width,
                               const uint64_t *ids, int64_t n, float *out,
                               void *plan_ws, void *pend, ha_stream_t stream);
int ha_sgd_push_pull_f32ids(float *table, int64_t rows, int64_t width,
                            void *plan_cur, int64_t n_cur, const float *grads, float lr,
                            void *pend_cur, const float *next_ids, int64_t n_next,
                            float *next_out, void *plan_next, void *pend_next,
                            ha_stream_t stream);
int ha_sgd_push_pull_u64ids(float *table, int64_t rows, int64_t width,
                            void *plan_cur, int64_t n_cur, const float *grads, float lr,
                            void *pend_cur, const uint64_t *next_ids, int64_t n_next,
                            float *next_out, void *plan_next, void *pend_next,
                            ha_stream_t stream);
int ha_debug_step_timeline(float *table, int64_t rows, int64_t width,
                           void *plan_cur, int64_t n_cur, const float *grads, float lr,
                           void *pend_cur, const float *next_ids, int64_t n_next,
                           float *next_out, void *plan_next, void *pend_next,
                           unsigned long long *dbg, ha_stream_t stream);
int64_t *ha_plan_handoff_timeout(void *plan_ws);

size_t ha_step_tab_bytes(void);
int64_t ha_step_max_ids(void);
int ha_step_tab_reset(void *tab, ha_stream_t stream);
int ha_step_f32ids(float *table, int64_t rows, int64_t width,
                   void *plan_cur, int64_t n_cur, const float *grads, float lr, const void *tab_cur,
                   void *plan_next, int64_t n_next, float *next_out, const void *tab_next,
                   void *plan_fin, int64_t n_fin, void *tab_fin,
                   const float *ahead_ids, int64_t n_ahead, void *plan_ahead,
                   void *tab_clear, ha_stream_t stream);
int ha_step_u64ids(float *table, int64_t rows, int64_t width,
                   void *plan_cur, int64_t n_cur, const float *grads, float lr, const void *tab_cur,
                   void *plan_next, int64_t n_next, float *next_out, const void *tab_next,
                   void *plan_fin, int64_t n_fin, void *tab_fin,
                   const uint64_t *ahead_ids, int64_t n_ahead, void *plan_ahead,
                   void *tab_clear, ha_stream_t stream);
int ha_debug_step_fwd_timeline(float *table, int64_t rows, int64_t width,
                               void *plan_cur, int64_t n_cur, const float *grads, float lr, const void *tab_cur,
                               void *plan_next, int64_t n_next, float *next_out, const void *tab_next,
                               void *plan_fin, int64_t n_fin, void *tab_fin,
                               const float *ahead_ids, int64_t n_ahead, void *plan_ahead,
                               void *tab_clear, unsigned long long *dbg, ha_stream_t stream);

int ha_qstep_init(void);
int64_t ha_qstep_max_ids(void);
size_t ha_qstep_queue_bytes(int64_t n_cap, int64_t width);
int ha_qplan_batch_f32ids(const float *const *ids, const int64_t *n, void *const *plans, int64_t count,
                          ha_stream_t stream);
int ha_qplan_batch_u64ids(const uint64_t *const *ids, const int64_t *n, void *const *plans, int64_t count,
                          ha_stream_t stream);
int ha_qqueue_batch(int64_t rows, int64_t width, void *const *plans_a, const int64_t *n_a, void *const *plans_g,
                    const int64_t *n_g, void *const *queues, int64_t queue_n_cap, int64_t count, ha_stream_t stream);
int ha_qapply(float *table, int64_t rows, int64_t width, void *plan_cur, int64_t n_cur, const float *grads, float lr,
              void *plan_next, int64_t n_next, float *next_out, const void *queue_cur, int64_t queue_n_cap,
              ha_stream_t stream);
int ha_qapply_sized(float *table, int64_t rows, int64_t width, void *plan_cur, int64_t n_cur, const float *grads,
                    float lr, void *plan_next, int64_t n_next, float *next_out, const void *queue_cur,
                    int64_t queue_n_cap, int64_t wave_items, ha_stream_t stream);
int ha_qapply_steps(float *table, int64_t rows, int64_t width, float lr, int64_t queue_n_cap, int64_t count,
                    void *const *plan_cur, const int64_t *n_cur, const float *const *grads, void *const *plan_next,
                    const int64_t *n_next, float *const *next_out, const void *const *queue_cur,
                    const int64_t *wave_items, ha_stream_t stream);
int ha_qqueue_batch_counts(int64_t rows, int64_t width, void *const *plans_a, const int64_t *n_a, void *const *plans_g,
                           const int64_t *n_g, void *const *queues, int64_t queue_n_cap, int64_t count,
                           uint32_t *const *counts_host, ha_stream_t stream);
void *ha_event_create(void);
int ha_event_destroy(void *event);
int ha_event_record(void *event, ha_stream_t stream);
int ha_stream_wait_event(ha_stream_t stream, void *event);
int ha_qqueue_batch_epochs(int64_t rows, int64_t width, void *const *plans_a, const int64_t *n_a, void *const *plans_g,
                           const int64_t *n_g, void *const *queues, int64_t queue_n_cap, int64_t count,
                           uint32_t *const *counts_host, const uint32_t *epochs, ha_stream_t stream);
int ha_qapply_steps_sync(float *table, int64_t rows, int64_t width, float lr, int64_t queue_n_cap, int64_t count,
                         void *const *plan_cur, const int64_t *n_cur, const float *const *grads, void *const *plan_next,
                         const int64_t *n_next, float *const *next_out, const void *const *queue_cur,
                         const int64_t *wave_items, const uint32_t *epochs, uint32_t *err, void *done_event,
                         ha_stream_t stream);
int ha_qapply_sync(float *table, int64_t rows, int64_t width, void *plan_cur, int64_t n_cur, const float *grads, float lr,
                   void *plan_next, int64_t n_next, float *next_out, const void *queue_cur, int64_t queue_n_cap,
                   int64_t wave_items, uint32_t epoch, uint32_t *err, void *done_event, ha_stream_t stream);
int ha_qapply_steps_counts(float *table, int64_t rows, int64_t width, float lr, int64_t queue_n_cap, int64_t count,
                           void *const *plan_cur, const int64_t *n_cur, const float *const *grads, void *const *plan_next,
                           const int64_t *n_next, float *const *next_out, const void *const *queue_cur,
                           const int64_t *wave_items, const uint32_t *const *counts_host, const uint32_t *epochs, uint32_t *err,
                           void *done_event, ha_stream_t stream);

int ha_xchg_available(void);
int ha_xchg_unique_id(void *id128);
void *ha_xchg_create(const void *id128, int world, int rank);
int ha_xchg_destroy(void *xchg);
int ha_xchg_bytes(void *xchg, const void *send, const int64_t *send_bytes, void *recv, const int64_t *recv_bytes,
                  ha_stream_t stream);
int ha_xchg_rows(void *xchg, const float *send, const int64_t *send_rows, float *recv, const int64_t *recv_rows, int64_t width,
                 ha_stream_t stream);

int64_t ha_qbig_max_ids(void);
size_t ha_qbig_plan_bytes(int64_t n_cap);
int ha_qbig_buckets(int64_t n_cap);
int ha_qbig_plan_batch_f32ids(const float *const *ids, const int64_t *n, void *const *ws, int64_t n_cap, int64_t count,
                              ha_stream_t stream);
int ha_qbig_plan_batch_u64ids(const uint64_t *const *ids, const int64_t *n, void *const *ws, int64_t n_cap, int64_t count,
                              ha_stream_t stream);
int ha_qbig_queue_batch(int64_t rows, int64_t width, void *const *ws_a, const int64_t *n_a, void *const *ws_g,
                        const int64_t *n_g, void *const *queues, int64_t n_cap, int64_t count, uint32_t *const *counts_host,
                        const uint32_t *epochs, ha_stream_t stream);
int ha_qbig_apply(float *table, int64_t rows, int64_t width, void *ws_cur, int64_t n_cur, const float *grads, float lr,
                  void *ws_next, int64_t n_next, float *next_out, const void *queue_cur, int64_t n_cap, int64_t coop_items,
                  uint32_t epoch, uint32_t *err, void *done_event, ha_stream_t stream);
int ha_qbig_plan_view(void *ws, int64_t n_cap, void **boff, void **bhdr, void **uniq, void **counts, void **seg, void **gperm,
                      void **meta);

int ha_qprep_f32ids(int64_t rows, int64_t width, const float *ahead_ids, int64_t n_ahead, void *plan_ahead,
                    void *plan_a, int64_t n_a, void *plan_g, int64_t n_g, void *queue_build, int64_t queue_n_cap,
                    ha_stream_t stream);
int ha_qprep_u64ids(int64_t rows, int64_t width, const uint64_t *ahead_ids, int64_t n_ahead, void *plan_ahead,
                    void *plan_a, int64_t n_a, void *plan_g, int64_t n_g, void *queue_build, int64_t queue_n_cap,
                    ha_stream_t stream);
int ha_qstep_f32ids(float *table, int64_t rows, int64_t width,
                    void *plan_cur, int64_t n_cur, const float *grads, float lr,
                    void *plan_next, int64_t n_next, float *next_out, const void *queue_cur,
                    void *plan_b1, int64_t n_b1, void *queue_build, int64_t queue_n_cap,
                    const float *ahead_ids, int64_t n_ahead, void *plan_ahead, ha_stream_t stream);
int ha_qstep_u64ids(float *table, int64_t rows, int64_t width,
                    void *plan_cur, int64_t n_cur, const float *grads, float lr,
                    void *plan_next, int64_t n_next, float *next_out, const void *queue_cur,
                    void *plan_b1, int64_t n_b1, void *queue_build, int64_t queue_n_cap,
                    const uint64_t *ahead_ids, int64_t n_ahead, void *plan_ahead, ha_stream_t stream);
const uint32_t *ha_qstep_queue_header(const void *queue);
int ha_debug_qapply(float *table, int64_t rows, int64_t width, void *plan_cur, int64_t n_cur, const float *grads,
                    float lr, void *plan_next, int64_t n_next, float *next_out, const void *queue_cur,
                    int64_t queue_n_cap, unsigned long long *dbg, ha_stream_t stream);
int ha_debug_qprep_f32ids(int64_t rows, int64_t width, const float *ahead_ids, int64_t n_ahead, void *plan_ahead,
                          void *plan_a, int64_t n_a, void *plan_g, int64_t n_g, void *queue_build, int64_t queue_n_cap,
                          unsigned long long *ph, ha_stream_t stream);

int ha_stream_gate(const uint32_t *flag, ha_stream_t stream);
int ha_debug_occupy(int64_t wgs, int64_t threads, int64_t lds_bytes, int64_t ticks, ha_stream_t stream);

int ha_sgd_apply_finish_prefetch_f32ids(float *table, int64_t rows, int64_t width,
                                        void *plan_ws, int64_t n, const float *grads, float lr,
                                        const float *next_ids, int64_t next_n, ha_stream_t stream);

int ha_shard_bucket(const void *plan_ws, int64_t n, const int64_t *starts_host,
                    int nshard, int32_t *offsets, uint32_t *local_keys,
                    ha_stream_t stream);

int ha_shard_route_f32ids(const float *ids, int64_t n, void *plan_ws,
                          const int64_t *starts_host, int nshard, int64_t *meta,
                          uint32_t *local_keys, ha_stream_t stream);
int ha_shard_route_u64ids(const uint64_t *ids, int64_t n, void *plan_ws,
                          const int64_t *starts_host, int nshard, int64_t *meta,
                          uint32_t *local_keys, ha_stream_t stream);

int ha_shard_route_pack_f32ids(const float *ids, int64_t n, void *plan_ws,
                               const int64_t *starts_host, int nshard, int64_t cap,
                               int64_t *meta, int32_t *send, ha_stream_t stream);
int ha_shard_route_pack_u64ids(const uint64_t *ids, int64_t n, void *plan_ws,
                               const int64_t *starts_host, int nshard, int64_t cap,
                               int64_t *meta, int32_t *send, ha_stream_t stream);
int ha_shard_route_unpack(const int32_t *recv, int nshard, int64_t cap, int64_t *recv_cnt,
                          uint32_t *keys_out, ha_stream_t stream);

int ha_shard_frames_route_f32ids(const float *ids, int64_t n, void *plan_ws, const int64_t *starts_host,
                                 int nshard, int64_t rcap, int64_t frame_stride, int32_t *send, int32_t *rowmap,
                                 int32_t *posmap, ha_stream_t stream);
int ha_shard_frames_route_u64ids(const uint64_t *ids, int64_t n, void *plan_ws, const int64_t *starts_host,
                                 int nshard, int64_t rcap, int64_t frame_stride, int32_t *send, int32_t *rowmap,
                                 int32_t *posmap, ha_stream_t stream);
int ha_shard_frames_pack(const void *plan_ws, int64_t n, const int64_t *starts_host, int nshard, int64_t rcap,
                         int64_t frame_stride, int32_t *send, int32_t *rowmap, int32_t *posmap, ha_stream_t stream);
int ha_shard_frames_unpack(const int32_t *recv, int nshard, int64_t rcap, int64_t frame_stride, uint32_t *keys_fixed,
                           int32_t *state, ha_stream_t stream);
int ha_shard_frames_pack_batch(const void *const *plan_ws, const int64_t *n, int count, const int64_t *starts_host,
                               int nshard, int64_t rcap, int64_t frame_stride, int32_t *send, int32_t *const *rowmap,
                               int32_t *const *posmap, ha_stream_t stream);
int ha_shard_frames_unpack_batch(const int32_t *recv, int count, int nshard, int64_t rcap, int64_t frame_stride,
                                 uint32_t *const *keys_fixed, int32_t *const *state, ha_stream_t stream);
int ha_shard_frames_serve_pull(const float *table, int64_t rows, int64_t width, const int32_t *recv, int nshard,
                               int64_t rcap, int64_t frame_stride, float *rows_out, uint32_t *keys_fixed,
                               int32_t *state, ha_stream_t stream);

int ha_shard_frames_pack_batch_sized(const void *const *plan_ws, const int64_t *n, int count, const int64_t *starts_host,
                                     int nshard, int self, int64_t rcap, int64_t frame_stride, int32_t *send,
                                     int32_t *const *rowmap, int32_t *const *posmap, int32_t *const *meta_dev,
                                     int32_t *const *meta_host, ha_stream_t stream);
int ha_shard_frames_unpack_batch_sized(const int32_t *recv, int count, int nshard, int64_t rcap, int64_t frame_stride,
                                       uint32_t *const *keys_fixed, int32_t *const *meta_dev, int32_t *const *meta_host,
                                       ha_stream_t stream);
int ha_shard_sized_serve_pull(const float *table, int64_t rows, int64_t width, const uint32_t *keys_fixed, int nshard,
                              int self, int64_t rcap, const int32_t *meta_dev, float *rows_out, ha_stream_t stream);
int ha_gather2_u32map(const float *table, int64_t rows, const float *recv, int64_t recv_rows, int64_t width,
                      const uint32_t *map, int64_t n, float *out, ha_stream_t stream);
int ha_shard_sized_serve_push(float *table, int64_t rows, int64_t width, const uint32_t *keys_fixed, int nshard, int self,
                              int64_t rcap, const int32_t *meta_dev, int64_t total, const float *push_buf, void *plan_ws,
                              ha_stream_t stream);
int ha_push_apply_scaled_finished(float *table, int64_t rows, int64_t width, void *plan_ws, int64_t n, const float *grads,
                                  float scale, ha_stream_t stream);

typedef struct ha_shard_slot {
    int32_t world, rank;
    int64_t rcap, n;
    void *plan_ws;
    const uint32_t *keys_fixed;
    const int32_t *meta_dev;
    const uint32_t *posmap;
    const int32_t *rowmap;
    const int32_t *counts_host;
    void *owner_plan_ws;
} ha_shard_slot;
int ha_shard_step_pull(const float *table, int64_t rows, int64_t width, const ha_shard_slot *slot, void *xchg, float *pull_send,
                       float *pull_recv, int64_t pull_rows, float *out, ha_stream_t stream);
int ha_shard_step_push(float *table, int64_t rows, int64_t width, const ha_shard_slot *slot, void *xchg, float *push_buf,
                       int64_t push_rows, const uint8_t *zero_flags, const float *values, float scale, ha_stream_t stream);
int ha_shard_step(float *table, int64_t rows, int64_t width, const ha_shard_slot *slot, void *xchg, float *pull_send,
                  float *pull_recv, int64_t pull_rows, float *push_buf, int64_t push_rows, const uint8_t *zero_flags, float *out,
                  const float *values, float scale, ha_stream_t stream);
int ha_shard_steps(float *table, int64_t rows, int64_t width, int64_t count, const ha_shard_slot *const *slots, void *xchg,
                   float *pull_send, float *pull_recv, int64_t pull_rows, float *push_buf, int64_t push_rows,
                   const uint8_t *zero_flags, float *const *outs, const float *const *values, float scale, ha_stream_t stream);

int ha_shard_serve_push(float *table, int64_t rows, int64_t width, const uint32_t *keys,
                        int64_t n, const float *values, void *plan_ws, ha_stream_t stream);

int ha_shard_frames_serve_push(float *table, int64_t rows, int64_t width, const uint32_t *keys_fixed, int nshard,
                               int64_t rcap, const float *values, void *plan_ws, ha_stream_t stream);

typedef struct ha_cache ha_cache;
ha_cache *ha_cache_create(int policy, int64_t limit, int64_t length,
                          int64_t width, int64_t max_batch);
void ha_cache_destroy(ha_cache *cache);
int ha_cache_set_bounds(ha_cache *cache, int64_t pull_bound, int64_t push_bound);
int ha_cache_set_bypass(ha_cache *cache, int bypass);
int ha_cache_bind_store(ha_cache *cache, float *table, int64_t *versions,
                        int64_t store_rows, int64_t row_start);
int ha_cache_lookup(ha_cache *cache, const void *keys, int key_kind, int64_t n,
                    float *dest, ha_stream_t stream);
int ha_cache_sort_ahead(ha_cache *cache, const void *keys, int key_kind, int64_t n, ha_stream_t stream);
int ha_cache_lookup_presorted(ha_cache *cache, const void *keys, int key_kind, int64_t n,
                              float *dest, ha_stream_t stream);
int ha_cache_sort_ahead_batch(ha_cache *cache, const void *const *keys, int key_kind, const int64_t *n, int count,
                              ha_stream_t stream);
int ha_cache_plan_block(ha_cache *cache, const void *const *keys, int key_kind, const int64_t *n, int count,
                        ha_stream_t side, ha_stream_t main);
int ha_cache_plan_block_push_keys(ha_cache *cache, const void *const *keys, int key_kind, const int64_t *n,
                                  const void *const *push_keys, int push_kind, const int64_t *n_push, int count,
                                  ha_stream_t side, ha_stream_t main);
int ha_cache_lookup_planned(ha_cache *cache, int64_t n, float *dest, ha_stream_t stream);
int ha_cache_update_planned(ha_cache *cache, int64_t n, const float *grads, ha_stream_t stream);
int ha_cache_plan_pending(ha_cache *cache);
int ha_cache_run_planned_pairs(ha_cache *cache, int count, const int64_t *n, float *const *dests, const float *const *grads,
                               ha_stream_t stream);
int ha_cache_plan_block_push_pull(ha_cache *cache, const void *const *keys, int key_kind, const int64_t *n, int count,
                                  ha_stream_t side, ha_stream_t main);
int ha_cache_push_pull_planned(ha_cache *cache, int64_t n_pull, float *dest, int64_t n_push, const float *grads,
                               ha_stream_t stream);
int ha_cache_run_planned_push_pulls(ha_cache *cache, int count, const int64_t *n_pull, float *const *dests,
                                    const int64_t *n_push, const float *const *grads, ha_stream_t stream);
int ha_cache_update(ha_cache *cache, const void *keys, int key_kind, int64_t n,
                    const float *grads, ha_stream_t stream);
int ha_cache_update_same_keys(ha_cache *cache, int64_t n, const float *grads, ha_stream_t stream);
int ha_cache_update_with_push_keys(ha_cache *cache, const void *keys,
                                   int key_kind, int64_t n,
                                   const void *push_keys, int push_kind,
                                   int64_t n_push, const float *grads,
                                   ha_stream_t stream);
int ha_cache_push_pull(ha_cache *cache, const void *pull_keys, int pull_kind,
                       int64_t n_pull, float *dest, const void *push_keys,
                       int push_kind, int64_t n_push, const float *grads,
                       ha_stream_t stream);
typedef struct {
    uint32_t *req_keys;
    int64_t *req_versions;
    int32_t *inbox_pull, *inbox_idx;
    int64_t *inbox_versions;
    float *inbox_rows;
    uint32_t *out_keys;
    int32_t *out_updates;
    float *out_rows;
    int64_t out_capacity, max_batch;
} ha_cache_remote;
int ha_cache_set_remote(ha_cache *cache);
int ha_cache_remote_buffers(ha_cache *cache, ha_cache_remote *out);
int ha_cache_lookup_begin(ha_cache *cache, const void *keys, int key_kind, int64_t n,
                          int64_t *n_unique_host, ha_stream_t stream);
int ha_cache_lookup_finish(ha_cache *cache, int64_t n, float *dest, ha_stream_t stream);
int ha_cache_outbox_count(ha_cache *cache, int64_t *count_host, ha_stream_t stream);
int ha_cache_outbox_pad(ha_cache *cache, int64_t entries);
int ha_cache_push_pull_begin(ha_cache *cache, const void *pull_keys, int pull_kind, int64_t n_pull,
                             const void *push_keys, int push_kind, int64_t n_push,
                             const float *grads, int64_t *n_unique_pull_host, ha_stream_t stream);
int ha_cache_push_pull_finish(ha_cache *cache, float *dest, ha_stream_t stream);
int ha_store_serve_sync(const float *table, const int64_t *server_versions, int64_t rows, int64_t width,
                        const uint32_t *keys, const int64_t *versions, int64_t m, int64_t bound,
                        int32_t *pull, int32_t *idx, int64_t *ver_out, float *rows_out,
                        int64_t *count_dev, void *scan_ws, ha_stream_t stream);
int ha_store_add_versions(int64_t *server_versions, int64_t rows, const uint32_t *keys,
                          const int32_t *updates, int64_t m, ha_stream_t stream);
int ha_store_push_distinct(float *table, int64_t *server_versions, int64_t rows, int64_t width, const uint32_t *keys,
                           const int32_t *updates, const float *grad_rows, int64_t m, ha_stream_t stream);
int ha_store_count_valid(const uint32_t *keys, int64_t m, int64_t rows, int64_t *acc, ha_stream_t stream);
int ha_cache_perf(ha_cache *cache, int64_t *out_host, ha_stream_t stream);
int ha_cache_state(ha_cache *cache, int64_t *out_host, ha_stream_t stream);
int ha_cache_phase_times(ha_cache *cache, uint64_t *out_host, ha_stream_t stream);
int ha_cache_set_timing(ha_cache *cache, int on);
int ha_cache_stage_times(ha_cache *cache, double *out_ms);
int ha_cache_snapshot(ha_cache *cache, int64_t cap, uint32_t *keys,
                      int64_t *version, int32_t *updates, uint64_t *stamp,
                      int32_t *slots, uint64_t *count_dev, ha_stream_t stream);
int ha_cache_set_line(ha_cache *cache, int64_t key, int64_t version, const float *data_dev, ha_stream_t stream);
float *ha_cache_data(ha_cache *cache);
float *ha_cache_grad(ha_cache *cache);
int64_t ha_cache_limit(ha_cache *cache);
int64_t ha_cache_width(ha_cache *cache);
int64_t ha_cache_fused_updates(ha_cache *cache);

typedef struct ha_laia ha_laia;
ha_laia *ha_laia_create(const uint64_t *samples_host, int64_t num_sample,
                        int64_t num_table, int64_t nrank, int64_t cache_size,
                        int64_t key_limit, int64_t max_batch);
void ha_laia_destroy(ha_laia *sched);
int ha_laia_next(ha_laia *sched, int64_t batch_id, int64_t mini_bs,
                 int64_t *dist_out, uint64_t *plan_out, int64_t plan_cap_elems,
                 int64_t *plan_off);
int ha_laia_hint_next(ha_laia *laia, int64_t next_batch_id);
int ha_laia_next_for_rank(ha_laia *h, int64_t batch_id, int64_t mini_bs, int64_t rank, int64_t *dist_out,
                          uint64_t *plan_out, int64_t plan_cap_elems, int64_t *plan_off);
int64_t ha_laia_snapshot_keys(ha_laia *sched, int64_t worker, int32_t *out,
                              int64_t cap);

int ha_laia_next_topk(ha_laia *sched, int64_t batch_id, int64_t mini_bs,
                      const int32_t *table_order, int64_t top_k, int64_t num_threads,
                      int64_t *dist_out, uint64_t *plan_out, int64_t plan_cap_elems,
                      int64_t *plan_off);
int ha_laia_counters(ha_laia *sched, int64_t *out);
int ha_laia_timing(ha_laia *h, double *out);
int ha_laia_timing_device(ha_laia *h, double *out);
int ha_laia_on_device(ha_laia *h);

typedef struct ha_shm_ring ha_shm_ring;
ha_shm_ring *ha_shm_ring_open(const char *name, int create, int64_t capacity_words);
void ha_shm_ring_close(ha_shm_ring *ring);
int ha_shm_ring_send(ha_shm_ring *ring, const uint64_t *words, int64_t n);
int64_t ha_shm_ring_recv(ha_shm_ring *ring, uint64_t *out, int64_t cap_words, int64_t *needed);
int64_t ha_shm_ring_pending_words(ha_shm_ring *ring);

int ha_debug_apply_timeline(float *table, int64_t rows, int64_t width,
                            const void *plan_ws, int64_t n, const float *grads,
                            float lr, unsigned long long *dbg,
                            ha_stream_t stream);

int ha_sgd_sparse_update_f32ids(float *table, int64_t rows, int64_t width,
                                const float *ids, int64_t n,
                                const float *grads, float lr,
                                ha_stream_t stream);

int ha_gather_sum_f32ids(const float *table, int64_t rows, int64_t width, const float *ids, int64_t n, int64_t bag,
                         const int64_t *offsets, int64_t nbags, float *out, ha_stream_t stream);
int ha_gather_sum_u64ids(const float *table, int64_t rows, int64_t width, const uint64_t *ids, int64_t n, int64_t bag,
                         const int64_t *offsets, int64_t nbags, float *out, ha_stream_t stream);
int ha_bag_of(const int64_t *offsets, int64_t nbags, int64_t n, int32_t *bag_of, ha_stream_t stream);
int ha_sgd_apply_bags(float *table, int64_t rows, int64_t width, const void *plan_ws, int64_t n, const float *bag_grads,
                      int64_t bag, const int32_t *bag_of, float lr, ha_stream_t stream);
int ha_sgd_sparse_update_bags_f32ids(float *table, int64_t rows, int64_t width, const float *ids, int64_t n,
                                     const float *bag_grads, int64_t bag, const int64_t *offsets, int64_t nbags, float lr,
                                     ha_stream_t stream);
int ha_sgd_sparse_update_bags_u64ids(float *table, int64_t rows, int64_t width, const uint64_t *ids, int64_t n,
                                     const float *bag_grads, int64_t bag, const int64_t *offsets, int64_t nbags, float lr,
                                     ha_stream_t stream);
int ha_debug_bag_slice(int floats);

typedef struct {
    int (*sparse_pull)(int node, const float *ids_dev, int64_t n, float *out_dev, void *stream);
    int (*sparse_push)(int node, const float *ids_dev, int64_t n, const float *vals_dev, void *stream);
    int (*barrier)(void);
} ha_ps_backend;
typedef struct {
    float *table;
    int64_t len, width, row_start, rows_local;
    void *stream;
} ha_ps_tensor_info;
int ha_ps_configure(int rank, int nrank);
int ha_ps_set_backend(const ha_ps_backend *backend);
int ha_ps_rank(void);
int ha_ps_nrank(void);
int ha_ps_init_tensor(int node, int ptype, int64_t len, int64_t width, int init_type,
                      double a, double b, uint64_t seed);
int ha_ps_attach_tensor(int node, float *table_dev, int64_t len, int64_t width);
int ha_ps_tensor(int node, ha_ps_tensor_info *out);
// ... 14 lines not shown
```

Measured before the change: 550.1 million.

## Fuse two consecutive apply steps into one paired queue kernel launch

Adds a pair-queue builder that classifies keys across three consecutive plans (current, next, after-next) so that two SGD apply steps plus the following lookup can be executed from one combined work queue. The apply path can now launch a paired kernel for even steps when the pair queue has been built and is flagged usable, and falls back to the single-step path otherwise. The aim is to halve the per-step launches and the table read/write traffic for rows touched in both steps. In exchange it adds an extra queue-build kernel, host polling of pair state with a short spin wait, and a substantially more complex code path.

```diff
diff --git a/herald_amd/_lib.py b/herald_amd/_lib.py
--- a/herald_amd/_lib.py
+++ b/herald_amd/_lib.py
@@ -123,6 +123,8 @@
     L.ha_qbig_buckets.argtypes = [i64]
     L.ha_qstep_queue_bytes.restype = sz
     L.ha_qstep_queue_bytes.argtypes = [i64, i64]
+    L.ha_qpair_queue_bytes.restype = sz
+    L.ha_qpair_queue_bytes.argtypes = [i64, i64]
     L.ha_qstep_queue_header.restype = vp
     L.ha_qstep_queue_header.argtypes = [vp]
     sigs = {
@@ -181,6 +183,8 @@
         "ha_shard_steps": [vp, i64, i64, i64, vp, vp, vp, vp, i64, vp, i64, vp, vp, vp, f32, vp],
         "ha_qapply_steps_sync": [vp, i64, i64, f32, i64, i64, vp, vp, vp, vp, vp, vp, vp, vp, vp, vp, vp, vp],
         "ha_qapply_steps_counts": [vp, i64, i64, f32, i64, i64, vp, vp, vp, vp, vp, vp, vp, vp, vp, vp, vp, vp, vp],
+        "ha_qpair_queue_batch": [i64, i64, vp, vp, vp, vp, vp, vp, vp, i64, i64, vp, vp, vp],
+        "ha_qapply_steps_pair": [vp, i64, i64, f32, i64, i64, vp, vp, vp, vp, vp, vp, vp, vp, vp, vp, vp, vp, vp, vp, vp],
         "ha_qapply_sync": [vp, i64, i64, vp, i64, vp, f32, vp, i64, vp, vp, i64, i64, c.c_uint32, vp, vp, vp],
         "ha_xchg_available": [],
         "ha_xchg_unique_id": [vp],
diff --git a/herald_amd/csrc/qpair_dev.h b/herald_amd/csrc/qpair_dev.h
--- /dev/null
+++ b/herald_amd/csrc/qpair_dev.h
@@ -0,0 +1,883 @@
+#pragma once
+
+namespace ha {
+
+struct QPHeader {
+    uint32_t n_coop[2], n_wave[2], n_copy;
+    uint32_t flags[3];
+    uint32_t epoch[3];
+    uint32_t verdict;
+    uint32_t n_class[2][4];
+    uint32_t reserved[44];
+};
+static_assert(sizeof(QPHeader) == 256, "pair queue header is one 256-byte line");
+struct QPEntry {
+    uint32_t w[16];
+};
+static_assert(sizeof(QPEntry) == 64, "pair queue items are 64 bytes");
+constexpr uint32_t kQPUnusable = 1u | 2u | 16u;
+
+struct QPLayout {
+    QPHeader *hdr;
+    QPEntry *coop0, *coop1, *wave0, *wave1, *copy;
+    uint32_t cap_coop, cap_wave0, cap_wave1, cap_copy;
+    size_t bytes;
+};
+static inline QPLayout qpair_layout(void *ws, int64_t n_cap, int64_t width) {
+    QPLayout q;
+    char *b = static_cast<char *>(ws);
+    const int64_t per512 = ceil_div(width, 512);
+    q.cap_coop = static_cast<uint32_t>(ceil_div(width, 64) * (2 * ceil_div(n_cap, kQLongC) + 2));
+    q.cap_wave0 = static_cast<uint32_t>(per512 * 3 * n_cap + 64);
+    q.cap_wave1 = static_cast<uint32_t>(per512 * 2 * n_cap + 64);
+    q.cap_copy = static_cast<uint32_t>(per512 * n_cap + 64);
+    q.hdr = reinterpret_cast<QPHeader *>(b);
+    q.coop0 = reinterpret_cast<QPEntry *>(b ? b + sizeof(QPHeader) : nullptr);
+    q.coop1 = q.coop0 ? q.coop0 + q.cap_coop : nullptr;
+    q.wave0 = q.coop1 ? q.coop1 + q.cap_coop : nullptr;
+    q.wave1 = q.wave0 ? q.wave0 + q.cap_wave0 : nullptr;
+    q.copy = q.wave1 ? q.wave1 + q.cap_wave1 : nullptr;
+    q.bytes = sizeof(QPHeader) +
+              (2 * static_cast<size_t>(q.cap_coop) + q.cap_wave0 + q.cap_wave1 + q.cap_copy) * sizeof(QPEntry);
+    return q;
+}
+
+__device__ __forceinline__ int qp_geo(uint32_t c1, uint32_t m1, uint32_t m2, bool in_table) {
+    if (!in_table)
+        return (m1 | m2) != 0u ? kQZ : kQNone;
+    const int k1 = q_kind(c1, m1, true), k2 = q_kind(m1, m2, true);
+    return k1 > k2 ? k1 : k2;
+}
+__device__ __forceinline__ int qp_slice(int geo) {
+    return geo == kQG ? 64 : geo == kQL ? 32 : geo == kQM ? 128 : 512;
+}
+__device__ __forceinline__ QCount qp_count(QCount t, int geo, uint32_t per512, uint32_t per128, uint32_t per64, uint32_t per32) {
+    t.g += geo == kQG ? per64 : 0u;
+    t.l += geo == kQL ? per32 : 0u;
+    t.m += geo == kQM ? per128 : 0u;
+    t.s += (geo == kQS || geo == kQZ) ? per512 : 0u;
+    return t;
+}
+
+constexpr int kQPairBatch = 8;
+struct QPairJob {
+    QPlan pa, pg, ph;
+    QPHeader *qh;
+    QPEntry *coop0, *coop1, *wave0, *wave1, *copy;
+    uint32_t *mirror;
+    uint32_t epoch;
+};
+struct QPairBatch {
+    int count, width;
+    uint64_t rows;
+    uint32_t cap_coop, cap_wave0, cap_wave1, cap_copy;
+    QPairJob job[kQPairBatch];
+};
+
+__device__ __forceinline__ uint32_t qp_probe(const uint32_t *tab, const uint32_t *keys, uint32_t key) {
+    uint32_t h = q_hash(key);
+    for (;;) {
+        const uint32_t e = tab[h];
+        if (e == kQTabEmpty || keys[e] == key)
+            return e;
+        h = (h + 1) & (kQTabSize - 1);
+    }
+}
+__device__ __forceinline__ void qp_insert(uint32_t *tab, const uint32_t *keys, int U, int tid) {
+    for (int y = tid; y < U; y += 1024) {
+        uint32_t h = q_hash(keys[y]);
+        for (;;) {
+            uint32_t seen = kQTabEmpty;
+            if (__hip_atomic_compare_exchange_strong(tab + h, &seen, static_cast<uint32_t>(y), __ATOMIC_RELAXED,
+                                                     __ATOMIC_RELAXED, __HIP_MEMORY_SCOPE_WORKGROUP))
+                break;
+            h = (h + 1) & (kQTabSize - 1);
+        }
+    }
+}
+__device__ __forceinline__ void qp_emit(QPEntry *dst, int geo, uint32_t key, uint32_t c1, uint32_t st1, uint32_t m1,
+                                        uint32_t fs1, uint32_t m2, uint32_t fs2, uint2 oa, uint2 og, int width) {
+    const int slice = qp_slice(geo);
+    int j = 0;
+    for (int col0 = 0; col0 < width; col0 += slice, ++j) {
+        uint4 q0, q1, q2;
+        q0.x = static_cast<uint32_t>(geo) | (static_cast<uint32_t>(col0 / 4) << 4);
+        q0.y = key;
+        q0.z = c1;
+        q0.w = st1;
+        q1.x = m1;
+        q1.y = fs1;
+        q1.z = m2;
+        q1.w = fs2;
+        q2.x = oa.x;
+        q2.y = oa.y;
+        q2.z = og.x;
+        q2.w = og.y;
+        q_st_item(reinterpret_cast<QEntry *>(dst + j), q0, q1);
+        q_st_item(reinterpret_cast<QEntry *>(dst + j) + 1, q2, uint4{0u, 0u, 0u, 0u});
+    }
+}
+
+struct QPKey {
+    uint32_t key, c1, st1, m1, fs1, m2, fs2;
+    uint2 oa, og;
+};
+__device__ __forceinline__ bool qp_key(const QPairJob &j, int part, uint32_t x, const uint32_t *tabX, const uint32_t *keysX,
+                                       const uint32_t *tabY, const uint32_t *keysY, bool full, QPKey *k) {
+    const QPlan &pi = part == 0 ? j.pa : part == 1 ? j.pg : j.ph;
+    k->key = pi.uniq[x];
+    const uint32_t cnt = static_cast<uint32_t>(pi.counts[x]);
+    const uint32_t ex = qp_probe(tabX, keysX, k->key), ey = qp_probe(tabY, keysY, k->key);
+    k->c1 = k->st1 = k->m1 = k->fs1 = k->m2 = k->fs2 = 0u;
+    k->oa = k->og = uint2{0u, 0u};
+    if (part == 0) {
+        k->c1 = cnt;
+        if (ex != kQTabEmpty)
+            k->m1 = static_cast<uint32_t>(j.pg.counts[ex]);
+        if (ey != kQTabEmpty)
+            k->m2 = static_cast<uint32_t>(j.ph.counts[ey]);
+        if (full) {
+            k->st1 = static_cast<uint32_t>(pi.seg[x]);
+            k->oa = reinterpret_cast<const uint2 *>(pi.occ)[x];
+            if (ex != kQTabEmpty) {
+                k->fs1 = static_cast<uint32_t>(j.pg.seg[ex]);
+                k->og = reinterpret_cast<const uint2 *>(j.pg.occ)[ex];
+            }
+            if (ey != kQTabEmpty)
+                k->fs2 = static_cast<uint32_t>(j.ph.seg[ey]);
+        }
+        return true;
+    }
+    if (part == 1) {
+        if (ex != kQTabEmpty)
+            return false;
+        k->m1 = cnt;
+        if (ey != kQTabEmpty)
+            k->m2 = static_cast<uint32_t>(j.ph.counts[ey]);
+        if (full) {
+            k->fs1 = static_cast<uint32_t>(pi.seg[x]);
+            k->og = reinterpret_cast<const uint2 *>(pi.occ)[x];
+            if (ey != kQTabEmpty)
+                k->fs2 = static_cast<uint32_t>(j.ph.seg[ey]);
+        }
+        return true;
+    }
+    if (ex != kQTabEmpty || ey != kQTabEmpty)
+        return false;
+    k->m2 = cnt;
+    if (full)
+        k->fs2 = static_cast<uint32_t>(pi.seg[x]);
+    return true;
+}
+
+__global__ __launch_bounds__(1024) void qpair_queue_kernel(const QPairBatch b) {
+    extern __shared__ __attribute__((aligned(16))) uint32_t s_dyn[];
+    const QPairJob &j = b.job[blockIdx.x / 3];
+    const int part = static_cast<int>(blockIdx.x % 3);
+    const int tid = static_cast<int>(threadIdx.x), w = tid >> 6;
+    const int Ua = uniform(j.pa.n > 0 ? static_cast<int>(j.pa.hdr->n_unique) : 0);
+    const int Ug = uniform(j.pg.n > 0 ? static_cast<int>(j.pg.hdr->n_unique) : 0);
+    const int Uh = uniform(j.ph.n > 0 ? static_cast<int>(j.ph.hdr->n_unique) : 0);
+    const int Ux = part == 0 ? Ug : Ua, Uy = part == 2 ? Ug : Uh, Ui = part == 0 ? Ua : part == 1 ? Ug : Uh;
+    const uint32_t *srcX = part == 0 ? j.pg.uniq : j.pa.uniq, *srcY = part == 2 ? j.pg.uniq : j.ph.uniq;
+    uint32_t *tabX = s_dyn, *tabY = s_dyn + kQTabSize, *keysX = tabY + kQTabSize, *keysY = keysX + Ux, *s_w = keysY + Uy;
+    for (int i = tid; i < 2 * kQTabSize; i += 1024)
+        s_dyn[i] = kQTabEmpty;
+    for (int y = tid; y < Ux; y += 1024)
+        keysX[y] = srcX[y];
+    for (int y = tid; y < Uy; y += 1024)
+        keysY[y] = srcY[y];
+    __syncthreads();
+    qp_insert(tabX, keysX, Ux, tid);
+    qp_insert(tabY, keysY, Uy, tid);
+    __syncthreads();
+    const uint32_t per512 = (b.width + 511) / 512, per128 = (b.width + 127) / 128, per64 = (b.width + 63) / 64,
+                   per32 = (b.width + 31) / 32;
+    QCount t{0u, 0u, 0u, 0u};
+    int bad = 0;
+    for (int x = tid; x < Ui; x += 1024) {
+        QPKey k;
+        if (!qp_key(j, part, static_cast<uint32_t>(x), tabX, keysX, tabY, keysY, false, &k))
+            continue;
+        const bool in_table = k.key < b.rows;
+        if (in_table && (k.c1 > kQChunk || k.m1 > kQChunk))
+            bad = 16;
+        t = qp_count(t, qp_geo(k.c1, k.m1, k.m2, in_table), per512, per128, per64, per32);
+    }
+    bad = __syncthreads_or(bad) ? 16 : 0;
+    uint32_t nL, nM, nS, nG;
+    QCount base;
+    base.l = qscan_n<16>(t.l, s_w, &nL, w);
+    base.m = qscan_n<16>(t.m, s_w, &nM, w) + nL;
+    base.s = qscan_n<16>(t.s, s_w, &nS, w) + nL + nM;
+    base.g = qscan_n<16>(t.g, s_w, &nG, w);
+    QPEntry *coop = part == 0 ? j.coop0 : j.coop1, *wave = part == 0 ? j.wave0 : part == 1 ? j.wave1 : j.copy;
+    const uint32_t cap_wave = part == 0 ? b.cap_wave0 : part == 1 ? b.cap_wave1 : b.cap_copy;
+    const uint32_t nW = nL + nM + nS;
+    uint32_t flags = static_cast<uint32_t>(bad);
+    if (nW > cap_wave || nG > b.cap_coop)
+        flags |= 1u;
+    if (part == 0 && ((j.pa.n > 0 && j.pa.hdr->reserved[kOrderFlagWord] != 0) ||
+                      (j.pg.n > 0 && j.pg.hdr->reserved[kOrderFlagWord] != 0) ||
+                      (j.ph.n > 0 && j.ph.hdr->reserved[kOrderFlagWord] != 0)))
+        flags |= 2u;
+    for (int x = tid; x < Ui; x += 1024) {
+        QPKey k;
+        if (!qp_key(j, part, static_cast<uint32_t>(x), tabX, keysX, tabY, keysY, true, &k))
+            continue;
+        const int geo = qp_geo(k.c1, k.m1, k.m2, k.key < b.rows);
+        if (geo == kQNone)
+            continue;
+        const uint32_t at = geo == kQG ? base.g : geo == kQL ? base.l : geo == kQM ? base.m : base.s;
+        const QCount nb = qp_count(base, geo, per512, per128, per64, per32);
+        const uint32_t cnt = (nb.g - base.g) + (nb.l - base.l) + (nb.m - base.m) + (nb.s - base.s);
+        if (at + cnt <= (geo == kQG ? b.cap_coop : cap_wave) && !(part == 2 && geo == kQG))
+            qp_emit((geo == kQG ? coop : wave) + at, geo, k.key, k.c1, k.st1, k.m1, k.fs1, k.m2, k.fs2, k.oa, k.og, b.width);
+        base = nb;
+    }
+    asm volatile("s_waitcnt vmcnt(0) lgkmcnt(0)" ::: "memory");
+    __syncthreads();
+    if (tid == 0) {
+        const uint32_t cw = min(nW, cap_wave), cg = min(nG, b.cap_coop);
+        if (part < 2) {
+            __hip_atomic_store(&j.qh->n_wave[part], cw, __ATOMIC_RELAXED, __HIP_MEMORY_SCOPE_AGENT);
+            __hip_atomic_store(&j.qh->n_coop[part], cg, __ATOMIC_RELAXED, __HIP_MEMORY_SCOPE_AGENT);
+            __hip_atomic_store(&j.qh->n_class[part][0], nG, __ATOMIC_RELAXED, __HIP_MEMORY_SCOPE_AGENT);
+            __hip_atomic_store(&j.qh->n_class[part][1], nL, __ATOMIC_RELAXED, __HIP_MEMORY_SCOPE_AGENT);
+            __hip_atomic_store(&j.qh->n_class[part][2], nM, __ATOMIC_RELAXED, __HIP_MEMORY_SCOPE_AGENT);
+            __hip_atomic_store(&j.qh->n_class[part][3], nS, __ATOMIC_RELAXED, __HIP_MEMORY_SCOPE_AGENT);
+        } else {
+            __hip_atomic_store(&j.qh->n_copy, cw, __ATOMIC_RELAXED, __HIP_MEMORY_SCOPE_AGENT);
+        }
+        __hip_atomic_store(&j.qh->flags[part], flags, __ATOMIC_RELAXED, __HIP_MEMORY_SCOPE_AGENT);
+        asm volatile("s_waitcnt vmcnt(0) lgkmcnt(0)" ::: "memory");
+        __hip_atomic_store(&j.qh->epoch[part], j.epoch, __ATOMIC_RELAXED, __HIP_MEMORY_SCOPE_AGENT);
+        if (j.mirror) {
+            j.mirror[part == 0 ? 3 : 5 + part] = flags;
+            if (part < 2)
+                j.mirror[4 + part] = cg + 1u;
+            __threadfence_system();
+            j.mirror[part] = cw + 1u;
+        }
+    }
+}
+
+static inline size_t qpair_lds_bytes(int n0, int n1, int n2) {
+    const int lo = n0 < n1 ? (n0 < n2 ? n0 : n2) : (n1 < n2 ? n1 : n2);
+    return 2 * kQTabSize * 4 + static_cast<size_t>(n0 + n1 + n2 - lo) * 4 + 32 * 4;
+}
+
+static int qpair_queue_batch(int64_t rows, int64_t width, void *const *plans_a, const int64_t *n_a, void *const *plans_g,
+                             const int64_t *n_g, void *const *plans_h, const int64_t *n_h, void *const *queues,
+                             int64_t queue_n_cap, int64_t count, uint32_t *const *counts_host, const uint32_t *epochs,
+                             hipStream_t stream) {
+    HA_REQUIRE(rows >= 0 && rows <= 0xFFFFFFFEll && width >= 4 && width % 4 == 0 && width <= (1 << 20),
+               "ha_qpair_queue_batch: rows of a multiple of 4 floats");
+    HA_REQUIRE(count >= 0 && (count == 0 || (plans_a && n_a && plans_g && n_g && plans_h && n_h && queues)),
+               "ha_qpair_queue_batch: null pointer");
+    HA_REQUIRE(count == 0 || (queue_n_cap >= 1 && queue_n_cap <= kQMax), "ha_qpair_queue_batch: bad queue capacity");
+    static DeviceOnce lds_allowed;
+    if (lds_allowed.run([]() -> int {
+            HA_ALLOW_LDS(qpair_queue_kernel, qpair_lds_bytes(kQMax, kQMax, kQMax));
+            return 0;
+        }))
+        return -1;
+    for (int64_t k0 = 0; k0 < count; k0 += kQPairBatch) {
+        QPairBatch b;
+        memset(&b, 0, sizeof(b));
+        b.rows = static_cast<uint64_t>(rows);
+        b.width = static_cast<int>(width);
+        size_t lds = 0;
+        for (int64_t k = k0; k < count && b.count < kQPairBatch; ++k) {
+            HA_REQUIRE(n_a[k] >= 0 && n_g[k] >= 0 && n_h[k] >= 0 && n_a[k] <= queue_n_cap && n_g[k] <= queue_n_cap &&
+                           n_h[k] <= queue_n_cap,
+                       "ha_qpair_queue_batch: a batch is larger than the queues were sized for");
+            HA_REQUIRE(queues[k] && (n_a[k] == 0 || plans_a[k]) && (n_g[k] == 0 || plans_g[k]) && (n_h[k] == 0 || plans_h[k]),
+                       "ha_qpair_queue_batch: null pointer (pair %lld)", (long long)k);
+            QPairJob &j = b.job[b.count++];
+            j.pa = qplan(plans_a[k], n_a[k]);
+            j.pg = qplan(plans_g[k], n_g[k]);
+            j.ph = qplan(plans_h[k], n_h[k]);
+            const QPLayout q = qpair_layout(queues[k], queue_n_cap, width);
+            j.qh = q.hdr;
+            j.coop0 = q.coop0;
+            j.coop1 = q.coop1;
+            j.wave0 = q.wave0;
+            j.wave1 = q.wave1;
+            j.copy = q.copy;
+            j.mirror = counts_host ? counts_host[k] : nullptr;
+            j.epoch = epochs ? epochs[k] : 0u;
+            b.cap_coop = q.cap_coop;
+            b.cap_wave0 = q.cap_wave0;
+            b.cap_wave1 = q.cap_wave1;
+            b.cap_copy = q.cap_copy;
+            const size_t need = qpair_lds_bytes(j.pa.n, j.pg.n, j.ph.n);
+            lds = lds > need ? lds : need;
+        }
+        hipLaunchKernelGGL(qpair_queue_kernel, dim3(3 * b.count), dim3(1024), lds, stream, b);
+        HA_LAUNCH_CHECK();
+    }
+    return 0;
+}
+
+struct QPArgs {
+    float *table;
+    uint64_t rows;
+    int width;
+    float lr;
+    const QPHeader *qh;
+    const QPEntry *coop0, *coop1, *wave0, *wave1, *copy;
+    uint32_t cap_coop, cap_wave0, cap_wave1, cap_copy;
+    const int32_t *perm_a, *perm_g, *perm_h;
+    const float *grads1, *grads2;
+    float *out1, *out2;
+    int ncoop, nworker;
+    uint32_t epoch;
+    uint32_t *err1, *err2;
+};
+struct QPItem {
+    int geo, col0, cols;
+    uint32_t key, c1, st1, m1, fs1, m2, fs2, oa0, oa1, og0, og1;
+};
+__device__ __forceinline__ QPItem qp_load(const QPEntry *e, int width) {
+    const uint4 q0 = reinterpret_cast<const uint4 *>(e)[0], q1 = reinterpret_cast<const uint4 *>(e)[1],
+                q2 = reinterpret_cast<const uint4 *>(e)[2];
+    QPItem it;
+    it.geo = static_cast<int>(uniform(q0.x & 15u));
+    it.col0 = static_cast<int>(uniform(q0.x >> 4)) * 4;
+    it.cols = min(qp_slice(it.geo), width - it.col0);
+    it.key = uniform(q0.y);
+    it.c1 = uniform(q0.z);
+    it.st1 = uniform(q0.w);
+    it.m1 = uniform(q1.x);
+    it.fs1 = uniform(q1.y);
+    it.m2 = uniform(q1.z);
+    it.fs2 = uniform(q1.w);
+    it.oa0 = uniform(q2.x);
+    it.oa1 = uniform(q2.y);
+    it.og0 = uniform(q2.z);
+    it.og1 = uniform(q2.w);
+    return it;
+}
+__device__ __forceinline__ uint32_t qp_occ(uint32_t o01, uint32_t o23, int t) {
+    return t == 0 ? (o01 & kQOccMask) : t == 1 ? (((o01 >> 21) | (o23 << 11)) & kQOccMask) : ((o23 >> 10) & kQOccMask);
+}
+
+__device__ __forceinline__ void qp_small_dests(float *out, const int32_t *perm, uint32_t fs, uint32_t m, int dv, int width,
+                                               int ca, int cb, bool a0, bool a1, float4v r0, float4v r1) {
+    const int lane = lane_id();
+    for (uint32_t j0 = 0; j0 < m; j0 += 64) {
+        if (j0 > 0)
+            dv = perm[fs + min(j0 + static_cast<uint32_t>(lane), m - 1u)];
+        const int cnt = static_cast<int>(min(64u, m - j0));
+        for (int j = 0; j < cnt; ++j) {
+            float *o = out + static_cast<uint64_t>(static_cast<uint32_t>(__builtin_amdgcn_readlane(dv, j))) *
+                                 static_cast<uint64_t>(width);
+            if (a0)
+                q_st_out(o + ca, r0);
+            if (a1)
+                q_st_out(o + cb, r1);
+        }
+    }
+}
+__device__ __forceinline__ void qp_small(const QPArgs &a, const QPItem &it) {
+    const int lane = lane_id();
+    const int width = a.width;
+    const int ca = it.col0 + 4 * lane, cb = ca + 256;
+    const bool a0 = 4 * lane < it.cols, a1 = 256 + 4 * lane < it.cols;
+    const int la = a0 ? ca : it.col0, lb = a1 ? cb : it.col0;
+    const bool zero = it.geo == kQZ;
+    const uint32_t c1 = zero ? 0u : it.c1, c2 = zero ? 0u : it.m1;
+    float *row = a.table + static_cast<uint64_t>(zero ? 0u : it.key) * static_cast<uint64_t>(width);
+    float4v r0{0.f, 0.f, 0.f, 0.f}, r1{0.f, 0.f, 0.f, 0.f};
+    if (!zero) {
+        r0 = q_ld_row<float4v>(row + la);
+        r1 = q_ld_row<float4v>(row + lb);
+    }
+    int dv1 = 0, dv2 = 0;
+    if (it.m1 > 3u)
+        dv1 = a.perm_g[it.fs1 + min(static_cast<uint32_t>(lane), it.m1 - 1u)];
+    else
+        dv1 = static_cast<int>(lane == 0 ? qp_occ(it.og0, it.og1, 0) : lane == 1 ? qp_occ(it.og0, it.og1, 1) : qp_occ(it.og0, it.og1, 2));
+    if (it.m2 > 0u)
+        dv2 = a.perm_h[it.fs2 + min(static_cast<uint32_t>(lane), it.m2 - 1u)];
+    float4v g0[kQSmallC], g1[kQSmallC], h0[kQSmallC], h1[kQSmallC];
+#pragma unroll
+    for (int t = 0; t < kQSmallC; ++t) {
+        if (static_cast<uint32_t>(t) < c1) {
+            const float *src = a.grads1 + static_cast<uint64_t>(qp_occ(it.oa0, it.oa1, t)) * static_cast<uint64_t>(width);
+            g0[t] = q_ld_grad<float4v>(src + la);
+            g1[t] = q_ld_grad<float4v>(src + lb);
+        }
+    }
+#pragma unroll
+    for (int t = 0; t < kQSmallC; ++t) {
+        if (static_cast<uint32_t>(t) < c1) {
+            r0 = sgd4(r0, g0[t], a.lr);
+            r1 = sgd4(r1, g1[t], a.lr);
+        }
+    }
+#pragma unroll
+    for (int t = 0; t < kQSmallC; ++t) {
+        if (static_cast<uint32_t>(t) < c2) {
+            const float *src = a.grads2 + static_cast<uint64_t>(qp_occ(it.og0, it.og1, t)) * static_cast<uint64_t>(width);
+            h0[t] = q_ld_grad<float4v>(src + la);
+            h1[t] = q_ld_grad<float4v>(src + lb);
+        }
+    }
+    qp_small_dests(a.out1, a.perm_g, it.fs1, it.m1, dv1, width, ca, cb, a0, a1, r0, r1);
+#pragma unroll
+    for (int t = 0; t < kQSmallC; ++t) {
+        if (static_cast<uint32_t>(t) < c2) {
+            r0 = sgd4(r0, h0[t], a.lr);
+            r1 = sgd4(r1, h1[t], a.lr);
+        }
+    }
+    if (c1 + c2 > 0u) {
+        if (a0)
+            q_st_row(row + ca, r0);
+        if (a1)
+            q_st_row(row + cb, r1);
+    }
+    qp_small_dests(a.out2, a.perm_h, it.fs2, it.m2, dv2, width, ca, cb, a0, a1, r0, r1);
+}
+
+__device__ __forceinline__ float2v_ qp_medium_chain(float2v_ r, const float *grads, int pidx, uint32_t c, int width, int lc,
+                                                    float lr) {
+    float2v_ g[kQMediumC];
+#pragma unroll
+    for (int t = 0; t < kQMediumC; ++t) {
+        const uint32_t o = static_cast<uint32_t>(__builtin_amdgcn_readlane(pidx, t));
+        g[t] = q_ld_grad<float2v_>(grads + static_cast<uint64_t>(o) * static_cast<uint64_t>(width) + lc);
+    }
+#pragma unroll
+    for (int t = 0; t < kQMediumC; ++t) {
+        const float x0 = __fsub_rn(r[0], __fmul_rn(lr, g[t][0]));
+        const float x1 = __fsub_rn(r[1], __fmul_rn(lr, g[t][1]));
+        const bool on = static_cast<uint32_t>(t) < c;
+        r[0] = on ? x0 : r[0];
+        r[1] = on ? x1 : r[1];
+    }
+    return r;
+}
+__device__ __forceinline__ void qp_medium_dests(float *out, const int32_t *perm, uint32_t fs, uint32_t m, int dv, int width,
+                                                int col, bool act, float2v_ r) {
+    const int lane = lane_id();
+    for (uint32_t j0 = 0; j0 < m; j0 += 64) {
+        if (j0 > 0)
+            dv = perm[fs + min(j0 + static_cast<uint32_t>(lane), m - 1u)];
+        const int cnt = static_cast<int>(min(64u, m - j0));
+        for (int j = 0; j < cnt; ++j) {
+            float *o = out + static_cast<uint64_t>(static_cast<uint32_t>(__builtin_amdgcn_readlane(dv, j))) *
+                                 static_cast<uint64_t>(width);
+            if (act)
+                q_st_out(o + col, r);
+        }
+    }
+}
+__device__ __forceinline__ void qp_medium(const QPArgs &a, const QPItem &it) {
+    const int lane = lane_id();
+    const int width = a.width;
+    const int col = it.col0 + 2 * lane;
+    const bool act = 2 * lane < it.cols;
+    const int lc = act ? col : it.col0;
+    float *row = a.table + static_cast<uint64_t>(it.key) * static_cast<uint64_t>(width);
+    int p1 = 0, p2 = 0, dv2 = 0;
+    if (it.c1 > 0u)
+        p1 = a.perm_a[it.st1 + min(static_cast<uint32_t>(lane), it.c1 - 1u)];
+    if (it.m1 > 0u)
+        p2 = a.perm_g[it.fs1 + min(static_cast<uint32_t>(lane), it.m1 - 1u)];
+    if (it.m2 > 0u)
+        dv2 = a.perm_h[it.fs2 + min(static_cast<uint32_t>(lane), it.m2 - 1u)];
+    float2v_ r = q_ld_row<float2v_>(row + lc);
+    if (it.c1 > 0u)
+        r = qp_medium_chain(r, a.grads1, p1, it.c1, width, lc, a.lr);
+    qp_medium_dests(a.out1, a.perm_g, it.fs1, it.m1, p2, width, col, act, r);
+    if (it.m1 > 0u)
+        r = qp_medium_chain(r, a.grads2, p2, it.m1, width, lc, a.lr);
+    if (it.c1 + it.m1 > 0u && act)
+        q_st_row(row + col, r);
+    qp_medium_dests(a.out2, a.perm_h, it.fs2, it.m2, dv2, width, col, act, r);
+}
+
+template <int Q>
+__device__ __forceinline__ float4v qp_chain4(float4v cur, const float *grads, const int32_t *perm, uint32_t st, uint32_t c,
+                                             int width, int col, float lr) {
+    constexpr int R = 64 / Q, NI = (kQMediumC + R - 1) / R;
+    const int lane = lane_id(), r = lane / Q, c4 = lane % Q;
+    const int pidx = perm[st + min(static_cast<uint32_t>(lane), c - 1u)];
+    float4v g[NI];
+#pragma unroll
+    for (int i = 0; i < NI; ++i) {
+        const uint32_t occ = static_cast<uint32_t>(r + R * i);
+        const uint32_t o = static_cast<uint32_t>(__shfl(pidx, static_cast<int>(min(occ, c - 1u)), 64));
+        g[i] = q_ld_grad<float4v>(grads + static_cast<uint64_t>(o) * static_cast<uint64_t>(width) + col);
+    }
+#pragma unroll
+    for (int t = 0; t < kQMediumC; ++t) {
+        float4v gv;
+#pragma unroll
+        for (int k = 0; k < 4; ++k)
+            gv[k] = __shfl(g[t / R][k], (t % R) * Q + c4, 64);
+        const float4v x = sgd4(cur, gv, lr);
+        cur = static_cast<uint32_t>(t) < c ? x : cur;
+    }
+    return cur;
+}
+__device__ __forceinline__ float4v qp_ltree8(float4v cur, const float *grads, const int32_t *perm, uint32_t st, uint32_t c,
+                                             int width, int col, float lr) {
+    const int lane = lane_id(), r = lane >> 3;
+    const int pidx = perm[st + min(static_cast<uint32_t>(lane), c - 1u)];
+    float4v g[8];
+#pragma unroll
+    for (int t = 0; t < 8; ++t) {
+        const uint32_t occ = static_cast<uint32_t>(8 * t + r);
+        const uint32_t o = static_cast<uint32_t>(__shfl(pidx, static_cast<int>(min(occ, c - 1u)), 64));
+        g[t] = q_ld_grad<float4v>(grads + static_cast<uint64_t>(o) * static_cast<uint64_t>(width) + col);
+    }
+    float4v p{0.f, 0.f, 0.f, 0.f};
+#pragma unroll
+    for (int t = 0; t < 8; ++t) {
+        const float4v q = acc4(p, g[t], lr);
+        p = static_cast<uint32_t>(8 * t + r) < c ? q : p;
+    }
+    p = add4(p, shfl_xor4(p, 8));
+    p = add4(p, shfl_xor4(p, 16));
+    p = add4(p, shfl_xor4(p, 32));
+    return sub4(cur, p);
+}
+__device__ __forceinline__ float4v qp_ltree16(float4v cur, const float *grads, const int32_t *perm, uint32_t st, uint32_t c,
+                                              int width, int col, float lr) {
+    const int lane = lane_id(), r = lane >> 4;
+    const int pidx = perm[st + min(static_cast<uint32_t>(lane), c - 1u)];
+    float4v half[2];
+#pragma unroll
+    for (int h = 0; h < 2; ++h) {
+        float4v g[8];
+#pragma unroll
+        for (int t = 0; t < 8; ++t) {
+            const uint32_t occ = static_cast<uint32_t>(8 * t + r + 4 * h);
+            const uint32_t o = static_cast<uint32_t>(__shfl(pidx, static_cast<int>(min(occ, c - 1u)), 64));
+            g[t] = q_ld_grad<float4v>(grads + static_cast<uint64_t>(o) * static_cast<uint64_t>(width) + col);
+        }
+        float4v p{0.f, 0.f, 0.f, 0.f};
+#pragma unroll
+        for (int t = 0; t < 8; ++t) {
+            const float4v q = acc4(p, g[t], lr);
+            p = static_cast<uint32_t>(8 * t + r + 4 * h) < c ? q : p;
+        }
+        p = add4(p, shfl_xor4(p, 16));
+        p = add4(p, shfl_xor4(p, 32));
+        half[h] = p;
+    }
+    return sub4(cur, add4(half[0], half[1]));
+}
+
+__device__ __forceinline__ void qp_long_dests(float *out, const int32_t *perm, uint32_t fs, uint32_t m, int width, int col,
+                                              bool act, float4v nv) {
+    const int lane = lane_id(), r = lane >> 3;
+    for (uint32_t j0 = 0; j0 < m; j0 += 64) {
+        const int dv = perm[fs + min(j0 + static_cast<uint32_t>(lane), m - 1u)];
+        const uint32_t cnt = min(64u, m - j0);
+        for (uint32_t j = 0; j < cnt; j += 8) {
+            const uint32_t d = static_cast<uint32_t>(__shfl(dv, static_cast<int>(min(j + r, cnt - 1u)), 64));
+            if (j + r < cnt && act)
+                q_st_out(out + static_cast<uint64_t>(d) * static_cast<uint64_t>(width) + col, nv);
+        }
+    }
+}
+__device__ __forceinline__ void qp_long(const QPArgs &a, const QPItem &it) {
+    const int lane = lane_id();
+    const int width = a.width;
+    const int r = lane >> 3, c4 = lane & 7;
+    const bool act = 4 * c4 < it.cols;
+    const int col = it.col0 + (act ? 4 * c4 : 0);
+    float *row = a.table + static_cast<uint64_t>(it.key) * static_cast<uint64_t>(width);
+    float4v cur = q_ld_row<float4v>(row + col);
+    if (it.c1 > static_cast<uint32_t>(kQMediumC))
+        cur = qp_ltree8(cur, a.grads1, a.perm_a, it.st1, it.c1, width, col, a.lr);
+    else if (it.c1 > 0u)
+        cur = qp_chain4<8>(cur, a.grads1, a.perm_a, it.st1, it.c1, width, col, a.lr);
+    qp_long_dests(a.out1, a.perm_g, it.fs1, it.m1, width, col, act, cur);
+    if (it.m1 > static_cast<uint32_t>(kQMediumC))
+        cur = qp_ltree8(cur, a.grads2, a.perm_g, it.fs1, it.m1, width, col, a.lr);
+    else if (it.m1 > 0u)
+        cur = qp_chain4<8>(cur, a.grads2, a.perm_g, it.fs1, it.m1, width, col, a.lr);
+    if (r == 0 && act)
+        q_st_row(row + col, cur);
+    qp_long_dests(a.out2, a.perm_h, it.fs2, it.m2, width, col, act, cur);
+}
+
+__device__ __forceinline__ float4v qp_coop_step(float4v cur, const float *grads, const int32_t *perm, uint32_t st, uint32_t c,
+                                                int width, int col, float lr, float *s_part) {
+    const int lane = lane_id(), w = uniform(static_cast<int>(threadIdx.x >> 6));
+    const int r = lane >> 4, c4 = lane & 15;
+    if (c == 0u)
+        return cur;
+    if (c < static_cast<uint32_t>(kQLongC)) {
+        if (w == 0) {
+            cur = c > static_cast<uint32_t>(kQMediumC) ? qp_ltree16(cur, grads, perm, st, c, width, col, lr)
+                                                       : qp_chain4<16>(cur, grads, perm, st, c, width, col, lr);
+            if (lane < 16)
+                *reinterpret_cast<float4v *>(s_part + 4 * c4) = cur;
+        }
+        __syncthreads();
+        cur = *reinterpret_cast<const float4v *>(s_part + 4 * c4);
+        __syncthreads();
+        return cur;
+    }
+    float4v p{0.f, 0.f, 0.f, 0.f};
+    for (uint32_t base = 0; base < c; base += 256) {
+        const uint32_t mine = base + 16u * static_cast<uint32_t>(w);
+        if (mine >= c)
+            break;
+        const int pidx = perm[st + min(mine + static_cast<uint32_t>(lane & 15), c - 1u)];
+        float4v g[4];
+#pragma unroll
+        for (int t = 0; t < 4; ++t) {
+            const uint32_t o = static_cast<uint32_t>(__shfl(pidx, 4 * t + r, 64));
+            g[t] = q_ld_grad<float4v>(grads + static_cast<uint64_t>(o) * static_cast<uint64_t>(width) + col);
+        }
+#pragma unroll
+        for (int t = 0; t < 4; ++t) {
+            const float4v q = acc4(p, g[t], lr);
+            p = mine + static_cast<uint32_t>(4 * t + r) < c ? q : p;
+        }
+    }
+    p = add4(p, shfl_xor4(p, 16));
+    p = add4(p, shfl_xor4(p, 32));
+    if (lane < 16)
+        *reinterpret_cast<float4v *>(s_part + w * 64 + 4 * c4) = p;
+    __syncthreads();
+    const float *sp = s_part + (4 * r) * 64 + 4 * c4;
+    float4v total = add4(add4(*reinterpret_cast<const float4v *>(sp), *reinterpret_cast<const float4v *>(sp + 64)),
+                         add4(*reinterpret_cast<const float4v *>(sp + 128), *reinterpret_cast<const float4v *>(sp + 192)));
+    total = add4(total, shfl_xor4(total, 16));
+    total = add4(total, shfl_xor4(total, 32));
+    __syncthreads();
+    return sub4(cur, total);
+}
+__device__ __forceinline__ void qp_coop_dests(float *out, const int32_t *perm, uint32_t fs, uint32_t m, int width, int col,
+                                              bool act, float4v nv) {
+    const int lane = lane_id(), w = uniform(static_cast<int>(threadIdx.x >> 6));
+    const int r = lane >> 4;
+    for (uint32_t k0 = 0; k0 * 64u < m; k0 += 16) {
+        const int dv = perm[fs + min(64u * (k0 + static_cast<uint32_t>(lane >> 2)) + static_cast<uint32_t>(4 * w + (lane & 3)),
+                                     m - 1u)];
+        const uint32_t rounds = min(16u, (m - 64u * k0 + 63u) / 64u);
+        for (uint32_t k = 0; k < rounds; ++k) {
+            const uint32_t j = 64u * (k0 + k) + static_cast<uint32_t>(4 * w + r);
+            const uint32_t d = static_cast<uint32_t>(__shfl(dv, static_cast<int>(4 * k) + r, 64));
+            if (j < m && act)
+                q_st_out(out + static_cast<uint64_t>(d) * static_cast<uint64_t>(width) + col, nv);
+        }
+    }
+}
+__device__ __forceinline__ void qp_coop(const QPArgs &a, const QPItem &it, float *s_part) {
+    const int lane = lane_id(), w = uniform(static_cast<int>(threadIdx.x >> 6));
+    const int width = a.width;
+    const int r = lane >> 4, c4 = lane & 15;
+    const bool act = 4 * c4 < it.cols;
+    const int col = it.col0 + (act ? 4 * c4 : 0);
+    float *row = a.table + static_cast<uint64_t>(it.key) * static_cast<uint64_t>(width);
+    float4v cur = q_ld_row<float4v>(row + col);
+    cur = qp_coop_step(cur, a.grads1, a.perm_a, it.st1, it.c1, width, col, a.lr, s_part);
+    qp_coop_dests(a.out1, a.perm_g, it.fs1, it.m1, width, col, act, cur);
+    cur = qp_coop_step(cur, a.grads2, a.perm_g, it.fs1, it.m1, width, col, a.lr, s_part);
+    if (w == 0 && r == 0 && act)
+        q_st_row(row + col, cur);
+    qp_coop_dests(a.out2, a.perm_h, it.fs2, it.m2, width, col, act, cur);
+}
+
+__global__ __launch_bounds__(kQWg, 8) void qapply_pair_kernel(const QPArgs a) {
+    extern __shared__ __attribute__((aligned(16))) uint32_t s_dyn[];
+    int b = blockIdx.x;
+    if (a.epoch != 0u) {
+        const uint32_t fail = ~a.epoch;
+        bool ready = a.qh->epoch[0] == a.epoch && a.qh->epoch[1] == a.epoch && a.qh->epoch[2] == a.epoch && a.qh->verdict != fail;
+        if (blockIdx.x == 0) {
+            const unsigned long long t_poll = __builtin_amdgcn_s_memrealtime();
+            for (int spin = 0; !ready && spin < (1 << 22); ++spin) {
+                const uint32_t e0 = __hip_atomic_load(&a.qh->epoch[0], __ATOMIC_ACQUIRE, __HIP_MEMORY_SCOPE_AGENT);
+                const uint32_t e1 = __hip_atomic_load(&a.qh->epoch[1], __ATOMIC_ACQUIRE, __HIP_MEMORY_SCOPE_AGENT);
+                const uint32_t e2 = __hip_atomic_load(&a.qh->epoch[2], __ATOMIC_ACQUIRE, __HIP_MEMORY_SCOPE_AGENT);
+                ready = uniform(static_cast<uint32_t>(e0 == a.epoch && e1 == a.epoch && e2 == a.epoch)) != 0u;
+                if (ready || __builtin_amdgcn_s_memrealtime() - t_poll > 200000000ull)
+                    break;
+                __builtin_amdgcn_s_sleep(64);
+            }
+            if (threadIdx.x == 0) {
+                __hip_atomic_store(const_cast<uint32_t *>(&a.qh->verdict), ready ? a.epoch : fail, __ATOMIC_RELAXED,
+                                   __HIP_MEMORY_SCOPE_AGENT);
+                if (!ready && a.err1 != nullptr)
+                    __hip_atomic_store(a.err1, 8u, __ATOMIC_RELAXED, __HIP_MEMORY_SCOPE_SYSTEM);
+                if (!ready && a.err2 != nullptr)
+                    __hip_atomic_store(a.err2, 8u, __ATOMIC_RELAXED, __HIP_MEMORY_SCOPE_SYSTEM);
+            }
+        } else if (!ready) {
+            const unsigned long long t_poll = __builtin_amdgcn_s_memrealtime();
+            uint32_t vd = 0u;
+            for (int spin = 0; spin < (1 << 23); ++spin) {
+                vd = uniform(__hip_atomic_load(&a.qh->verdict, __ATOMIC_ACQUIRE, __HIP_MEMORY_SCOPE_AGENT));
+                if (vd == a.epoch || vd == fail || __builtin_amdgcn_s_memrealtime() - t_poll > 400000000ull)
+                    break;
+                __builtin_amdgcn_s_sleep(64);
+            }
+            ready = vd == a.epoch;
+            if (!ready && vd != fail && threadIdx.x == 0) {
+                if (a.err1 != nullptr)
+                    __hip_atomic_store(a.err1, 8u, __ATOMIC_RELAXED, __HIP_MEMORY_SCOPE_SYSTEM);
+                if (a.err2 != nullptr)
+                    __hip_atomic_store(a.err2, 8u, __ATOMIC_RELAXED, __HIP_MEMORY_SCOPE_SYSTEM);
+            }
+        }
+        if (!ready)
+            return;
+    }
+    if (((a.qh->flags[0] | a.qh->flags[1] | a.qh->flags[2]) & kQPUnusable) != 0u) {
+        if (blockIdx.x == 0 && threadIdx.x == 0) {
+            if (a.err1 != nullptr)
+                __hip_atomic_store(a.err1, 8u, __ATOMIC_RELAXED, __HIP_MEMORY_SCOPE_SYSTEM);
+            if (a.err2 != nullptr)
+                __hip_atomic_store(a.err2, 8u, __ATOMIC_RELAXED, __HIP_MEMORY_SCOPE_SYSTEM);
+        }
+        return;
+    }
+    if (b < a.ncoop) {
+        const uint32_t g0 = min(a.qh->n_coop[0], a.cap_coop), n = g0 + min(a.qh->n_coop[1], a.cap_coop);
+        for (uint32_t e = static_cast<uint32_t>(b); e < n; e += static_cast<uint32_t>(a.ncoop)) {
+            const QPItem it = qp_load(e < g0 ? a.coop0 + e : a.coop1 + (e - g0), a.width);
+            qp_coop(a, it, reinterpret_cast<float *>(s_dyn));
+        }
+        return;
+    }
+    b -= a.ncoop;
+    const uint32_t w0 = min(a.qh->n_wave[0], a.cap_wave0), n0 = w0 + min(a.qh->n_wave[1], a.cap_wave1);
+    const uint32_t n1 = min(a.qh->n_copy, a.cap_copy), n = n0 + n1;
+    const uint32_t stride = static_cast<uint32_t>(a.nworker) * static_cast<uint32_t>(kQWpw);
+    const uint32_t wv = uniform(static_cast<uint32_t>(threadIdx.x >> 6));
+    const uint32_t both = 2u * (n0 < n1 ? n0 : n1);
+    for (uint32_t e = static_cast<uint32_t>(b) * static_cast<uint32_t>(kQWpw) + wv; e < n; e += stride) {
+        uint32_t i;
+        bool cp;
+        if (e < both) {
+            cp = (e & 1u) != 0u;
+            i = e >> 1;
+        } else {
+            cp = n0 <= n1;
+            i = n0 > n1 ? e - n1 : e - n0;
+        }
+        const QPEntry *src = cp ? a.copy + i : i < w0 ? a.wave0 + i : a.wave1 + (i - w0);
+        const QPItem it = qp_load(src, a.width);
+        if (it.geo == kQL)
+            qp_long(a, it);
+        else if (it.geo == kQM)
+            qp_medium(a, it);
+        else
+            qp_small(a, it);
+    }
+}
+
+static int qapply_pair(float *table, int64_t rows, int64_t width, float lr, void *plan_a, int64_t n_a, const float *grads1,
+                       void *plan_g, int64_t n_g, float *out1, const float *grads2, void *plan_h, int64_t n_h, float *out2,
+                       const void *pair_queue, int64_t queue_n_cap, int64_t wave_items, uint32_t epoch, uint32_t *err1,
+                       uint32_t *err2, hipEvent_t done, hipStream_t stream) {
+    HA_REQUIRE(table != nullptr && rows >= 0 && rows <= 0xFFFFFFFEll && width >= 4 && width % 4 == 0 &&
+                   width <= (1 << 20) && reinterpret_cast<uintptr_t>(table) % 16 == 0,
+               "ha_qapply_steps_pair: the table must be 16-byte aligned with rows of a multiple of 4 floats");
+    HA_REQUIRE(pair_queue != nullptr && queue_n_cap >= 1 && queue_n_cap <= kQMax && n_a >= 0 && n_g >= 0 && n_h >= 0 &&
+                   n_a <= queue_n_cap && n_g <= queue_n_cap && n_h <= queue_n_cap,
+               "ha_qapply_steps_pair: no more ids per batch than the pair queue was sized for");
+    HA_REQUIRE(n_a == 0 || (plan_a && grads1 && reinterpret_cast<uintptr_t>(grads1) % 16 == 0),
+               "ha_qapply_steps_pair: the first batch needs its plan and 16-byte aligned gradients");
+    HA_REQUIRE(n_g == 0 || (plan_g && grads2 && out1 && reinterpret_cast<uintptr_t>(grads2) % 16 == 0 &&
+                            reinterpret_cast<uintptr_t>(out1) % 16 == 0),
+               "ha_qapply_steps_pair: the second batch needs its plan, 16-byte aligned gradients and output");
+    HA_REQUIRE(n_h == 0 || (plan_h && out2 && reinterpret_cast<uintptr_t>(out2) % 16 == 0),
+               "ha_qapply_steps_pair: the third batch needs its plan and a 16-byte aligned output");
+    QPArgs a;
+    memset(&a, 0, sizeof(a));
+    a.table = table;
+    a.rows = static_cast<uint64_t>(rows);
+    a.width = static_cast<int>(width);
+    a.lr = lr;
+    const QPLayout q = qpair_layout(const_cast<void *>(pair_queue), queue_n_cap, width);
+    a.qh = q.hdr;
+    a.coop0 = q.coop0;
+    a.coop1 = q.coop1;
+    a.wave0 = q.wave0;
+    a.wave1 = q.wave1;
+    a.copy = q.copy;
+    a.cap_coop = q.cap_coop;
+    a.cap_wave0 = q.cap_wave0;
+    a.cap_wave1 = q.cap_wave1;
+    a.cap_copy = q.cap_copy;
+    a.perm_a = n_a > 0 ? plan_layout(plan_a, n_a).perm : nullptr;
+    a.perm_g = n_g > 0 ? plan_layout(plan_g, n_g).perm : nullptr;
+    a.perm_h = n_h > 0 ? plan_layout(plan_h, n_h).perm : nullptr;
+    a.grads1 = grads1;
+    a.grads2 = grads2;
+    a.out1 = out1;
+    a.out2 = out2;
+    a.epoch = epoch;
+    a.err1 = err1;
+    a.err2 = err2;
+    a.ncoop = (n_a >= kQLongC || n_g >= kQLongC) ? kQCoopSlots : 0;
+    const int64_t bound = static_cast<int64_t>(ceil_div(width, 512)) * (n_a + n_g + n_h);
+    a.nworker = static_cast<int>(bound / kQWpw + 1 < kQWorkerMax ? bound / kQWpw + 1 : kQWorkerMax);
+    if (wave_items >= 0 && wave_items / kQWpw + 1 < a.nworker)
+        a.nworker = static_cast<int>(wave_items / kQWpw + 1);
+    if (done != nullptr)
+        hipExtLaunchKernelGGL(qapply_pair_kernel, dim3(static_cast<unsigned>(a.ncoop + a.nworker)), dim3(kQWg), kQWpw * 64 * 4,
+                              stream, nullptr, done, 0, a);
+    else
+        hipLaunchKernelGGL(qapply_pair_kernel, dim3(static_cast<unsigned>(a.ncoop + a.nworker)), dim3(kQWg), kQWpw * 64 * 4,
+                           stream, a);
+    HA_LAUNCH_CHECK();
+    return 0;
+}
+
+}
+
+extern "C" size_t ha_qpair_queue_bytes(int64_t n_cap, int64_t width) {
+    if (n_cap < 1 || n_cap > ha::kQMax || width < 4 || width > (1 << 20))
+        return 0;
+    return ha::qpair_layout(nullptr, n_cap, width).bytes;
+}
+extern "C" int ha_qpair_queue_batch(int64_t rows, int64_t width, void *const *plans_a, const int64_t *n_a,
+                                    void *const *plans_g, const int64_t *n_g, void *const *plans_h, const int64_t *n_h,
+                                    void *const *pair_queues, int64_t queue_n_cap, int64_t count,
+                                    uint32_t *const *counts_host, const uint32_t *epochs, ha_stream_t stream) {
+    return ha::qpair_queue_batch(rows, width, plans_a, n_a, plans_g, n_g, plans_h, n_h, pair_queues, queue_n_cap, count,
+                                 counts_host, epochs, as_stream(stream));
+}
+extern "C" int ha_qapply_steps_pair(float *table, int64_t rows, int64_t width, float lr, int64_t queue_n_cap, int64_t count,
+                                    void *const *plan_cur, const int64_t *n_cur, const float *const *grads,
+                                    void *const *plan_next, const int64_t *n_next, float *const *next_out,
+                                    const void *const *queue_cur, const int64_t *wave_items, const uint32_t *epochs,
+                                    uint32_t *const *errs, const void *const *pair_queue, const uint32_t *pair_epochs,
+                                    const int64_t *pair_items, void *done_event, ha_stream_t stream) {
+    HA_REQUIRE(count >= 0 && (count == 0 || (plan_cur && n_cur && grads && plan_next && n_next && next_out && queue_cur)),
+               "ha_qapply_steps_pair: null pointer");
+    hipEvent_t done = static_cast<hipEvent_t>(done_event);
+    for (int64_t k = 0; k < count; ++k) {
+        if (pair_queue && pair_queue[k] && k + 1 < count) {
+            HA_REQUIRE(plan_next[k] == plan_cur[k + 1] && n_next[k] == n_cur[k + 1],
+                       "ha_qapply_steps_pair: steps %lld and %lld do not share their middle batch", (long long)k, (long long)k + 1);
+            if (ha::qapply_pair(table, rows, width, lr, plan_cur[k], n_cur[k], grads[k], plan_next[k], n_next[k], next_out[k],
+                                grads[k + 1], plan_next[k + 1], n_next[k + 1], next_out[k + 1], pair_queue[k], queue_n_cap,
+                                pair_items ? pair_items[k] : -1, pair_epochs ? pair_epochs[k] : 0u, errs ? errs[k] : nullptr,
+                                errs ? errs[k + 1] : nullptr, k + 2 == count ? done : nullptr, as_stream(stream)))
+                return -1;
+            ++k;
+            continue;
+        }
+        if (ha::qapply(table, rows, width, plan_cur[k], n_cur[k], grads[k], lr, plan_next[k], n_next[k], next_out[k],
+                       queue_cur[k], queue_n_cap, as_stream(stream), nullptr, wave_items ? wave_items[k] : -1,
+                       epochs ? epochs[k] : 0u, errs ? errs[k] : nullptr, k + 1 == count ? done : nullptr))
+            return -1;
+    }
+    if (count == 0 && done)
+        HA_CHECK_HIP(hipEventRecord(done, as_stream(stream)));
+    return 0;
+}
diff --git a/herald_amd/csrc/qstep.hip b/herald_amd/csrc/qstep.hip
--- a/herald_amd/csrc/qstep.hip
+++ b/herald_amd/csrc/qstep.hip
@@ -2314,3 +2314,5 @@
 extern "C" const uint32_t *ha_qstep_queue_header(const void *queue) {
     return reinterpret_cast<const uint32_t *>(queue);
 }
+
+#include "qpair_dev.h"
diff --git a/herald_amd/ops.py b/herald_amd/ops.py
--- a/herald_amd/ops.py
+++ b/herald_amd/ops.py
@@ -730,7 +730,7 @@
 
 class QueueStepPipeline:
 
-    def __init__(self, table, capacity, lr, device=None, block=8, overlap=True, sync="events", min_flags_block=8):
+    def __init__(self, table, capacity, lr, device=None, block=8, overlap=True, sync="events", min_flags_block=8, pair=None):
         L = _lib.load()
         _require(table, torch.float32, "table")
         self.table, self.lr = table, float(lr)
@@ -782,6 +782,24 @@
         self._ev_pool = []
         self._last_items = 0
         self.fallbacks, self._fb_plan, self._wide_ids = 0, None, {}
+        can_pair = self.overlap and not self.wide and table.shape[1] > 128 and self.block >= 2 and self.block % 2 == 0
+        if pair is None:
+            pair = can_pair and os.environ.get("HA_QPAIR", "1") != "0"
+        elif pair and not can_pair:
+            raise ValueError("pair=True needs overlap, batches of at most %d ids, rows wider than 128 floats and an even block"
+                             % qstep_max_ids())
+        self.pair = bool(pair)
+        self.pair_launches = self.pair_fallbacks = 0
+        if self.pair:
+            self.NPQUEUE = self.block
+            self.pqueue_bytes = int(L.ha_qpair_queue_bytes(self.capacity, table.shape[1]))
+            self.pqueues = torch.zeros(self.NPQUEUE * self.pqueue_bytes, dtype=torch.uint8, device=self.device)
+            torch.cuda.current_stream(self.device).synchronize()
+            self._pqueue_ptr = [self.pqueues.data_ptr() + q * self.pqueue_bytes for q in range(self.NPQUEUE)]
+            self.pcounts = torch.zeros((self.COUNTS, 8), dtype=torch.int32).pin_memory()
+            self._pcounts_c = (ctypes.c_int32 * (self.COUNTS * 8)).from_address(self.pcounts.data_ptr())
+            self._pcounts_base = self.pcounts.data_ptr()
+            self._pair_wait = True
         self._enq_last = None
         self.reset()
 
@@ -935,6 +953,27 @@
             else:
                 check(L.ha_qqueue_batch_epochs(rows, width, pa, na, pg, ng, qs, self.capacity, cnt, cs, eps, sp),
                       "ha_qqueue_batch")
+        if self.pair:
+            pairs = [p for p in range((b + 1) * B // 2, (b + 2) * B // 2) if nget(2 * p, 0) or nget(2 * p + 1, 0)]
+            pcc, pring = self._pcounts_c, self.COUNTS
+            for p in range((b + 1) * B // 2, (b + 2) * B // 2):
+                at = 8 * (p % pring)
+                for i in range(8):
+                    pcc[at + i] = 0
+                if p not in pairs:
+                    pcc[at + 3] = 32
+                    pcc[at] = pcc[at + 1] = pcc[at + 2] = 1
+            if pairs:
+                cnt = len(pairs)
+                pp, NP = self._plan_ptr, self.NPLAN
+                trip = [[(pp[(2 * p + d) % NP] if nget(2 * p + d, 0) else None) for p in pairs] for d in range(3)]
+                ntrip = [[nget(2 * p + d, 0) for p in pairs] for d in range(3)]
+                pqs = (vp * cnt)(*[self._pqueue_ptr[p % self.NPQUEUE] for p in pairs])
+                pcs = (vp * cnt)(*[self._pcounts_base + 32 * (p % pring) for p in pairs])
+                peps = (ctypes.c_uint32 * cnt)(*[self._pair_epoch(p) for p in pairs])
+                check(L.ha_qpair_queue_batch(rows, width, (vp * cnt)(*trip[0]), (i64 * cnt)(*ntrip[0]), (vp * cnt)(*trip[1]),
+                                             (i64 * cnt)(*ntrip[1]), (vp * cnt)(*trip[2]), (i64 * cnt)(*ntrip[2]), pqs,
+                                             self.capacity, cnt, pcs, peps, sp), "ha_qpair_queue_batch")
         if self.overlap and not flags:
             ev = self._event()
             ev.record(s)
@@ -950,6 +989,21 @@
     @staticmethod
     def _epoch(j):
         return (j + (1 << 24)) & 0xFFFFFFFF
+
+    @staticmethod
+    def _pair_epoch(p):
+        return (p + (1 << 25)) & 0xFFFFFFFF
+
+    def pair_state(self, p, wait=0.0):
+        import time
+        at = 8 * (p % self.COUNTS)
+        cc = self._pcounts_c
+        if wait > 0.0 and not (cc[at] and cc[at + 1] and cc[at + 2]):
+            t0 = time.perf_counter()
+            while not (cc[at] and cc[at + 1] and cc[at + 2]) and time.perf_counter() - t0 < wait:
+                pass
+        built = bool(cc[at] and cc[at + 1] and cc[at + 2])
+        return built, cc[at + 3] | cc[at + 6] | cc[at + 7], (cc[at] + cc[at + 1] + cc[at + 2] - 3) if built else -1
 
     def _block_done_event(self, c):
         if self.sync != "flags" or (c + 1) % self.block != 0:
@@ -1081,9 +1135,12 @@
         vp, i64 = ctypes.c_void_p, ctypes.c_int64
         pc = (vp * cnt)(*[self.plan_of(c0 + i).ws.data_ptr() for i in range(cnt)])
         pn = (vp * cnt)(*[self.plan_of(c0 + i + 1).ws.data_ptr() for i in range(cnt)])
-        ns = (i64 * cnt)(*[n] * cnt)
-        gs = (vp * cnt)(*[g.data_ptr() for g in grads_list])
-        os_ = (vp * cnt)(*[o.data_ptr() for o in out_list])
+        sizes = [int(x) for x in n] if hasattr(n, "__len__") else [int(n)] * (cnt + 1)
+        if len(sizes) != cnt + 1:
+            raise ValueError("apply_steps_call: n must be one size or the sizes of %d batches" % (cnt + 1))
+        ns, nn = (i64 * cnt)(*sizes[:cnt]), (i64 * cnt)(*sizes[1:])
+        gs = (vp * cnt)(*[g.data_ptr() if g is not None else None for g in grads_list])
+        os_ = (vp * cnt)(*[o.data_ptr() if o is not None else None for o in out_list])
         qs = (vp * cnt)(*[self._queue(c0 + i) for i in range(cnt)])
         hints = (i64 * cnt)(*[-1] * cnt)
         head = (vp(t.data_ptr()), i64(rows), i64(width), ctypes.c_float(self.lr), i64(self.capacity), i64(cnt))
@@ -1097,6 +1154,21 @@
         cs = (vp * cnt)()
         base = self._counts_base
         use_counts = os.environ.get("HA_QCOUNTS", "0") != "0"
+        pair = self.pair and sized and not torch.cuda.is_current_stream_capturing()
+        if pair:
+            def span(x):
+                return x.data_ptr(), x.data_ptr() + x.numel() * x.element_size()
+
+            def apart(*ts):
+                sp_ = sorted(span(x) for x in ts if x is not None and x.numel())
+                return all(sp_[i][1] <= sp_[i + 1][0] for i in range(len(sp_) - 1))
+            pair_ok = [i + 1 < cnt and apart(out_list[i], out_list[i + 1], grads_list[i], grads_list[i + 1]) for i in range(cnt)]
+            pq = (vp * cnt)()
+            peps = (ctypes.c_uint32 * cnt)()
+            pitems = (i64 * cnt)(*[-1] * cnt)
+            errs = (vp * cnt)()
+            fn_pair = L.ha_qapply_steps_pair
+            pair_epoch, pqueue_ptr, NPQ = self._pair_epoch, self._pqueue_ptr, self.NPQUEUE
 
         def call(k0):
             if flags and k0 // B != (k0 + cnt - 1) // B:
@@ -1114,14 +1186,39 @@
                         self._last_items = w + cp - 2
                     hints[i] = w + cp - 2 if w > 0 and cp > 0 else (self._last_items * 17) // 16 if self._last_items > 0 else -1
                     cs[i] = base + 4 * at if use_counts else None
-            if flags:
+            if pair:
+                for i in range(cnt):
+                    pq[i] = None
+                    if (k0 + i) % 2 or not pair_ok[i]:
+                        continue
+                    p = (k0 + i) // 2
+                    built, fl, items = self.pair_state(p, 0.0)
+                    if built:
+                        self._pair_wait = True
+                    elif self._pair_wait:
+                        built, fl, items = self.pair_state(p, 0.05)
+                        self._pair_wait = built
+                    if built and not fl:
+                        pq[i] = pqueue_ptr[p % NPQ]
+                        peps[i] = pair_epoch(p) if flags else 0
+                        pitems[i] = items
+                        self.pair_launches += 1
+                    else:
+                        self.pair_fallbacks += 1
+                for i in range(cnt):
+                    eps[i] = epoch(k0 + i) if flags else 0
+                    errs[i] = base + 16 * ((k0 + i) % ring) + 12 if flags else None
+                done = self._block_done_event(k0 + cnt - 1) if flags else None
+                if fn_pair(*head, pc, ns, gs, pn, nn, os_, qs, hints, eps, errs, pq, peps, pitems, done, sp) != 0:
+                    check(-1, "ha_qapply_steps_pair")
+            elif flags:
                 for i in range(cnt):
                     eps[i] = epoch(k0 + i)
                 done = self._block_done_event(k0 + cnt - 1)
-                if fn_sync(*head, pc, ns, gs, pn, ns, os_, qs, hints, cs if sized else None, eps, last_err(k0 + cnt - 1), done,
+                if fn_sync(*head, pc, ns, gs, pn, nn, os_, qs, hints, cs if sized else None, eps, last_err(k0 + cnt - 1), done,
                            sp) != 0:
                     check(-1, "ha_qapply_steps_counts")
-            elif fn(*head, pc, ns, gs, pn, ns, os_, qs, hints, sp) != 0:
+            elif fn(*head, pc, ns, gs, pn, nn, os_, qs, hints, sp) != 0:
                 check(-1, "ha_qapply_steps")
         return call
 
diff --git a/include/herald_amd.h b/include/herald_amd.h
--- a/include/herald_amd.h
+++ b/include/herald_amd.h
@@ -299,6 +299,17 @@
                            const int64_t *n_next, float *const *next_out, const void *const *queue_cur,
                            const int64_t *wave_items, const uint32_t *const *counts_host, const uint32_t *epochs, uint32_t *err,
                            void *done_event, ha_stream_t stream);
+size_t ha_qpair_queue_bytes(int64_t n_cap, int64_t width);
+int ha_qpair_queue_batch(int64_t rows, int64_t width, void *const *plans_a, const int64_t *n_a, void *const *plans_g,
+                         const int64_t *n_g, void *const *plans_h, const int64_t *n_h, void *const *pair_queues,
+                         int64_t queue_n_cap, int64_t count, uint32_t *const *counts_host, const uint32_t *epochs,
+                         ha_stream_t stream);
+int ha_qapply_steps_pair(float *table, int64_t rows, int64_t width, float lr, int64_t queue_n_cap, int64_t count,
+                         void *const *plan_cur, const int64_t *n_cur, const float *const *grads, void *const *plan_next,
+                         const int64_t *n_next, float *const *next_out, const void *const *queue_cur,
+                         const int64_t *wave_items, const uint32_t *epochs, uint32_t *const *errs,
+                         const void *const *pair_queue, const uint32_t *pair_epochs, const int64_t *pair_items,
+                         void *done_event, ha_stream_t stream);
 
 int ha_xchg_available(void);
 int ha_xchg_unique_id(void *id128);
```

Measured after the change: 507.3 million. 7.8% lower.
